# ywq/psnerf

Measured on AMD Instinct MI355X. Metric: ray-samples/sec (train step) on BEAR stage2, higher is better.
Workload: dtype f32

## Files before the change

include/psnerf_hip.h:

```cpp
#ifndef PSNERF_HIP_H
#define PSNERF_HIP_H

#include <stdint.h>

#ifdef __cplusplus
extern "C" {
#endif

#define PSN_OK 0
#define PSN_E_ARG (-1)
#define PSN_E_LAUNCH (-2)
#define PSN_E_UNSUPPORTED (-3)

const char* psn_last_error(void);
int psn_version(void);

int psn_composite_fwd(const float* alpha, const float* rgb, int64_t n_rays, int n_samples, int white_bg,
                      float* weights, float* rgb_out, float* acc_out, void* stream);
int psn_composite_bwd(const float* alpha, const float* rgb, const float* d_rgb_out, const float* d_acc_out,
                      int64_t n_rays, int n_samples, int white_bg, float* d_alpha, float* d_rgb, void* stream);

int psn_pe_encode(const float* x, int64_t n, int n_freqs, float scale, float* out, int out_stride, void* stream);
int psn_app_input(const float* p, const float* v, const float* normal, int64_t n, int n_freqs, float* out, void* stream);

// ... 161 lines not shown
    const float* const* mask_ptrs; const float* const* aux2_ptrs; float* const* save2_ptrs;
    const float* act_init; int64_t act_init_rows; const float* rk_coef; const float* rk_basis; int rk_k; const uint32_t* dump_tiles;
    int64_t n_rows; float* out; const float* live_count; int64_t live_period;
} PsnMlpLaunch;
typedef struct { int chain, width16, src, trim, from_a, x3, tb_lds, pm_groups; int64_t blocks, pm_period; } PsnMlpPath;
int psn_mlp_launch(const PsnMlpDesc* desc, const float* packed_w, const float* packed_b, const PsnMlpLaunch* launch, PsnMlpPath* path,
                   void* stream);
int psn_mlp_last_path(PsnMlpPath* path);
int psn_mlp_block_order(int point_major);

#define PSN_SCATTER_MAX_ITEMS 16
typedef struct {
    const float* rows;
    float* dense;
    int64_t row_stride, col_stride;
    int B, C;
    float fill;
} PsnScatterItem;
int psn_scatter_rows(int n_items, const PsnScatterItem* items, const int* inv, int64_t N, int64_t Ns, void* stream);
int psn_gather_rows(int n_items, const PsnScatterItem* items, const int64_t* idx, int64_t N, int64_t Ns, void* stream);
int psn_gather_rows_valid(int n_items, const PsnScatterItem* items, const int64_t* idx, const int* inv, int64_t N, int64_t Ns, void* stream);

int psn_secant_step(const float* occ, float tau, float* d_pred, float* d_low, float* d_high, float* f_low, float* f_high,
                    const float* origin, const float* dir, float* p_mid, int64_t n, void* stream);

int psn_first_crossing(const float* occ, const float* far, const float* u, const float* omu, float near, float tau,
                       int64_t n_rays, int n_steps, float* bracket, int* flags, void* stream);

int psn_shadow_points(const float* surf, const float* ldir, int64_t n_surf, int n_lights, int n_steps, float lnear, float lfar,
                      const float* u, const float* omu, float box, float* pts, int64_t* rows, unsigned long long* counter,
                      void* stream);

int psn_mlp_infer_pe(const PsnMlpDesc* desc, const float* packed_w, const float* packed_b, const float* points, int64_t n_rows,
                     int pe_octaves, float pe_scale, float* out, void* stream);
int psn_mlp_infer_pe_indirect(const PsnMlpDesc* desc, const float* packed_w, const float* packed_b, const float* points,
                              int64_t capacity, const long long* n_rows_dev, const int64_t* out_rows, int pe_octaves,
                              float pe_scale, float* out, void* stream);

int psn_march_sweep(const PsnMlpDesc* desc, const float* packed_w, const float* packed_b, const float* origin, const float* dir,
                    const float* far, const float* u, const float* omu, float near, int64_t n_rays, int n_steps, float tau,
                    int pe_octaves, float pe_scale, int* skip, unsigned long long* n_blocks, float* occ, void* stream);

int psn_root_find(const PsnMlpDesc* desc, const float* packed_w, const float* packed_b, const float* origin, const float* dir,
                  const float* bracket, int64_t n_rays, float tau, int n_iter, int pe_octaves, float pe_scale, float* d_out,
                  void* stream);

int psn_stage2_loss_fwd(const float* rgb, const float* rgb_gt, int L, const float* alb, const float* alb_j, const float* wgt,
                        const float* wgt_j, int nb, const float* vis, const float* vis_gt, int V, const float* nrm,
                        const float* nrm_gt, const float* nrm_j, const unsigned char* mask_a, const unsigned char* mask_b,
                        int64_t N, int l2, const float* inv_denom, const float* weight, const float* count_dev, float* partial,
                        float* out, void* stream);
int psn_stage2_loss_bwd(const float* g_total, const float* rgb, const float* rgb_gt, int L, float k_rgb, float* d_rgb,
                        const float* alb, const float* alb_j, float k_alb, float* d_alb, float* d_alb_j, const float* wgt,
                        const float* wgt_j, int nb, float k_wgt, float* d_wgt, float* d_wgt_j, const float* vis, const float* vis_gt,
                        int V, float k_vis, float* d_vis, const float* nrm, const float* nrm_gt, const float* nrm_j, float k_nrm,
                        float k_nrmj, float* d_nrm, float* d_nrm_j, const unsigned char* mask_a, const unsigned char* mask_b,
                        int64_t N, int l2, const float* count_dev, void* stream);

int psn_stage1_loss_partial_floats(void);
int psn_stage1_loss_fwd(const float* rgb, const float* rgb_gt, const float* diff, const unsigned char* hit, const float* normal,
                        const float* normal_gt, const unsigned char* norm_mask, const float* acc, const float* mask_gt,
                        const unsigned char* mask_valid, int64_t N, int64_t n_rays, const float* weights, float* partial,
                        float* sums, float* terms, void* stream);
int psn_stage1_loss_terms(const float* sums, int64_t n_rays, const float* weights, int has_grad, int has_norm, int has_mask,
                          float* terms, void* stream);
int psn_stage1_loss_bwd(const float* g_loss, const float* sums, const float* rgb, const float* rgb_gt, const unsigned char* hit,
                        const float* normal, const float* normal_gt, const unsigned char* norm_mask, const float* acc,
                        const float* mask_gt, const unsigned char* mask_valid, int64_t N, int64_t n_rays, const float* weights,
                        float* d_rgb, float* d_diff, float* d_normal, float* d_acc, void* stream);
int psn_surface_normals_fwd(const float* g, const unsigned char* hit, int64_t N, float eps, float* norm_pred, float* diff,
                            void* stream);
int psn_surface_normals_bwd(const float* g, const unsigned char* hit, int64_t N, float eps, const float* d_norm_pred,
                            const float* d_diff, float* dg, void* stream);

#define PSN_PAIR_SUMS_MAX_V 16
#define PSN_PAIR_SUMS_MAX_CHUNKS 2048
int psn_pair_sums(const float* x, int V, int64_t Ns, int C, float* sx, float* sl_part, int* n_chunks, void* stream);
#define PSN_PAIR_GROUP_MAX 4
typedef struct { const float* x; float* sx; float* dWl; float* bias; } PsnPairSumsItem;
int64_t psn_pair_sums_group_workspace(int n_items, int V, int64_t Ns, int C);
int psn_pair_sums_group(int n_items, const PsnPairSumsItem* items, int V, int64_t Ns, int C, const float* pe_l, int64_t ld_pe, int n_pe,
                        int64_t ld_w, float* workspace, void* stream);

#define PSN_ROW_ADAM_MAX 4
typedef struct {
    float* param; const float* grad; float* exp_avg; float* exp_avg_sq;
    int64_t rows; int cols;
    float one_minus_beta1, one_minus_beta2, eps, step_size;
} PsnRowAdamItem;
int psn_row_adam(int n_items, const PsnRowAdamItem* items, const int64_t* idx, int n_idx, void* stream);
int psn_row_adam_dev(int n_items, const PsnRowAdamItem* items, const int64_t* idx, int n_idx, const float* step_sizes_dev, void* stream);

int psn_normalize_rows_fwd(const float* x, int64_t n, float eps, float* y, void* stream);
int psn_normalize_rows_bwd(const float* x, const float* g, int64_t n, float eps, float* dx, void* stream);
int psn_light_rows_fwd(const float* dir_table, const float* int_table, const int64_t* idx, int n_idx, float eps, float* dir_out,
                       float* int_out, void* stream);
int psn_light_rows_bwd(const float* dir_table, const int64_t* idx, int n_idx, int64_t n_rows, float eps, const float* g_dir,
                       const float* g_int, float* d_dir_table, float* d_int_table, void* stream);
int psn_camera_rays(const float* uv, const float* pose, const float* intrinsics, const int64_t* idx, int64_t n, float scale,
                    float* out, void* stream);
int psn_stage1_rays(const float* pix, const float* camera_mat, int k_ld, const float* world_mat, float radius2, int64_t n,
                    float* cam, float* rays, float* far, void* stream);
int psn_surface_points(const float* d_pred, const int* flags, const float* cam, const float* rays, int64_t n, float* d_i,
                       float* dists, unsigned char* obj_mask, float* points, void* stream);
int psn_stage1_targets(const float* pix, int64_t n, int h, int w, const float* img, const float* mask, const float* mask_valid,
                       const float* normal, const float* norm_mask, const float* world_mat, int use_angle, float cos_thresh,
                       float* rgb_gt, float* mask_gt, unsigned char* mask_valid_out, float* normal_gt,
                       unsigned char* norm_mask_out, void* stream);
#define PSN_COPY2D_MAX 24
typedef struct {
    const float* src; int64_t ld_src;
    float* dst; int64_t ld_dst;
    int rows, cols;
} PsnCopy2dItem;
int psn_copy2d_group(int n_items, const PsnCopy2dItem* items, void* stream);
#define PSN_COPY_BYTES_MAX 24
typedef struct { const void* src; void* dst; int64_t n_bytes; int aligned; } PsnCopyBytesItem;
int psn_copy_bytes_group(int n_items, const PsnCopyBytesItem* items, void* stream);
int psn_mask_count(const unsigned char* mask_a, const unsigned char* mask_b, int64_t n, float* out, void* stream);
int psn_surface_index(const unsigned char* mask, int64_t n, int64_t cap, int64_t* idx, float* count, void* stream);
int psn_inverse_index(const int64_t* idx, int64_t ns, int64_t n_pix, int* inv, const float* count, void* stream);
typedef struct {
    const void* images; int image_type; const float* lut;
    const unsigned char* object_mask; const unsigned char* surface_mask;
    const float* points; const float* normal; const float* visibility; const float* vis_plus; const float* light_direction;
    int64_t hw; int width;
    const int64_t* lidx; int n_lights;
    const int64_t* pix; int64_t pix0; int64_t n;
    const int64_t* vidx; int n_vis;
    float* rgb; unsigned char* object_mask_out; unsigned char* surface_mask_out; float* uv; float* points_out; float* normal_out;
    float* visibility_out; float* vis_train_gt; int64_t* sampling_idx_out; float* light_direction_out;
} PsnViewBatch;
int psn_view_batch(const PsnViewBatch* b, void* stream);
#define PSN_ADAM_MAX_SEGS 16
typedef struct {
    int64_t offset, grad_offset, n;
    float neg_step_size;
    float bias_correction2_sqrt;
} PsnAdamSeg;
int psn_adam_flat(float* param, const float* grad, float* exp_avg, float* exp_avg_sq, int n_segs, const PsnAdamSeg* segs,
                  float one_minus_beta1, float beta2, float one_minus_beta2, float eps, void* stream);
int psn_adam_flat_dev(float* param, const float* grad, float* exp_avg, float* exp_avg_sq, int n_segs, const PsnAdamSeg* segs,
                      float one_minus_beta1, float beta2, float one_minus_beta2, float eps, const float* seg_scalars_dev, void* stream);

#define PSN_WN_MAX_ITEMS 16
typedef struct {
    const float* v;
    const float* g;
    float* w;
    const float* dw;
    float* dv;
    float* dg;
    int rows, cols;
    float scale;
} PsnWnItem;
int psn_weight_norm_fwd(int n_items, const PsnWnItem* items, void* stream);
int psn_weight_norm_bwd(int n_items, const PsnWnItem* items, void* stream);

typedef struct {
    int32_t n_hidden;
    int32_t n_out;
    int32_t out_act;
    int32_t reserved;
    uint8_t has_in[PSN_MLP_MAX_LAYERS + 4];
} PsnBf16Desc;

// ... 132 lines not shown
```

psnerf_amd/csrc/gemm.hip:

```cpp
#include "common.h"

namespace psn {

constexpr int BM = 128, BK = 16, LDA = BM + 4, EPI_LD = 68;

struct GemmArgs {
    int64_t M;
    int N, K;
    const float* A;
    int64_t lda;
    const float* B;
    int64_t ldb;
    float* C;
    int64_t ldc;
    const float* bias;
    int epi;
    const float* aux_in;
    int64_t ld_aux_in;
    const float* aux_in2;
    int64_t ld_aux_in2;
    float* aux_out;
    int64_t ld_aux_out;
    int k_chunk;
    int tiles_n;
    int64_t n_tiles;
    int split_k;
    int a_vec, b_vec;
    int c_vec, auxin_vec, auxin2_vec, auxout_vec;
    int64_t split_stride;
    float* colsum;
    const float* A2;
    int64_t lda2;
    const float* B2;
    int64_t ldb2;
    int seg_splits;
    int b_div, b_mod;
    const float* Bt2;
    int64_t ldbt2;
    int b2_div, b2_mod, b_split;
};

__device__ __forceinline__ int fastdiv24(int k, int d) {
    int q = (int)((float)k * __builtin_amdgcn_rcpf((float)d));
    const int r = k - q * d;
    q += (r >= d ? 1 : 0) - (r < 0 ? 1 : 0);
    return q;
}

template <bool KCONTIG, int ROWS>
__device__ __forceinline__ void fetch_tile(const float* __restrict__ src, int64_t ld, int64_t row0, int64_t n_rows,
                                           int k0, int k_end, int vec_ok, int tid, float4 (&v)[ROWS / 64],
                                           int k_div = 0, int k_mod = 0, const float* __restrict__ src2 = nullptr,
                                           int64_t ld2 = 0, int k_div2 = 0, int k_mod2 = 0, int col_split = 0) {
#pragma unroll
    for (int u = 0; u < ROWS / 64; ++u) {
        int f = tid + 256 * u;
        float4 x = make_float4(0.f, 0.f, 0.f, 0.f);
        if (KCONTIG) {
            int r = f >> 2, kq = (f & 3) * 4;
            int64_t row = row0 + r;
            int k = k0 + kq;
            if (row < n_rows) {
                const float* p = src + row * ld + k;
                if (vec_ok && k + 3 < k_end) {
                    x = *reinterpret_cast<const float4*>(p);
                } else {
                    if (k + 0 < k_end) x.x = p[0];
                    if (k + 1 < k_end) x.y = p[1];
                    if (k + 2 < k_end) x.z = p[2];
                    if (k + 3 < k_end) x.w = p[3];
                }
            }
        } else {
            int kk = f / (ROWS / 4), rq = (f % (ROWS / 4)) * 4;
            int k = k0 + kk;
            int64_t row = row0 + rq;
            if (k < k_end) {
                const bool second = col_split > 0 && row >= col_split;
                const int kd = second ? k_div2 : k_div, km = second ? k_mod2 : k_mod;
                int ks = k;
                if (kd > 0) {
                    if (k_end <= (1 << 24)) {
                        if (kd > 1) ks = fastdiv24(k, kd);
// ... 201 lines not shown
#pragma unroll
            for (int e = 0; e < 4; ++e) {
                float x = vv[e];
                switch (epi) {
                    case PSN_EPI_NONE: break;
                    case PSN_EPI_BIAS: x = x + bb[e]; break;
                    case PSN_EPI_BIAS_RELU: x = fmaxf(x + bb[e], 0.0f); break;
                    case PSN_EPI_BIAS_SOFTPLUS: { float sp, sg; softplus100_sig(x + bb[e], sp, sg); x = sp; o2[e] = sg; break; }
                    case PSN_EPI_MUL_AUX: x = x * a1[e]; break;
                    case PSN_EPI_MUL_POS: x = a1[e] > 0.0f ? x : 0.0f; break;
                    case PSN_EPI_BIAS_SIGMOID: x = sigmoidf_(x + bb[e]); break;
                    case PSN_EPI_ACCUM: x = cin[e] + x; break;
                    case PSN_EPI_MUL2: o2[e] = x * a2[e]; x = x * a1[e]; break;
                    case PSN_EPI_SOFTPLUS_BWD: x = a1[e] * (x + 100.0f * a2[e] * (1.0f - a1[e])); break;
                    case PSN_EPI_MUL_AUX_RAW: o2[e] = x; x = x * a1[e]; break;
                    default: break;
                }
                vv[e] = x;
            }
            if (full4 && g.c_vec) *reinterpret_cast<float4*>(cp) = make_float4(vv[0], vv[1], vv[2], vv[3]);
            else { for (int e = 0; e < 4; ++e) if (nbase + e < g.N) cp[e] = vv[e]; }
            if (has_o2) {
                float* op = g.aux_out + m * g.ld_aux_out + nbase;
                if (full4 && g.auxout_vec) *reinterpret_cast<float4*>(op) = make_float4(o2[0], o2[1], o2[2], o2[3]);
                else { for (int e = 0; e < 4; ++e) if (nbase + e < g.N) op[e] = o2[e]; }
            }
        }
        __builtin_amdgcn_fence(__ATOMIC_ACQ_REL, "wavefront");
        __builtin_amdgcn_wave_barrier();
    }
    }
}

template <bool TA, bool TB, int NT>
__global__ __launch_bounds__(256) void gemm_kernel(GemmArgs g) {
    __shared__ __attribute__((aligned(16))) float lds_raw[GemmLds<NT>::FLOATS];
    gemm_tile<TA, TB, NT>(g, blockIdx.x, lds_raw);
}

constexpr int kMaxGroup = PSN_GEMM_TN_MAX_ITEMS;
struct GroupedArgs {
    int n;
    int64_t block_start[kMaxGroup + 1];
    GemmArgs g[kMaxGroup];
};
__global__ __launch_bounds__(256) void gemm_tn_grouped_kernel(GroupedArgs gg) {
    __shared__ __attribute__((aligned(16))) float lds_raw[GemmLds<2>::FLOATS];
    int i = 0;
    while (i + 1 < gg.n && (int64_t)blockIdx.x >= gg.block_start[i + 1]) ++i;
    const GemmArgs g = gg.g[i];
    const int64_t bid = (int64_t)blockIdx.x - gg.block_start[i];
    if (bid >= g.n_tiles * (int64_t)g.split_k) return;
    gemm_tile<true, false, 2>(g, bid, lds_raw);
}

template <int NU>
__device__ __forceinline__ void fetch_tile256(const float* __restrict__ src, int64_t ld, int n_rows, int k0, int k_end,
                                              int tid, float4 (&v)[NU]) {
    const int rqc = min((tid & 63) * 4, ((n_rows - 1) >> 2) << 2);
    const int wave = __builtin_amdgcn_readfirstlane(tid >> 6);
#pragma unroll
    for (int u = 0; u < NU; ++u) {
        const int kc = min(k0 + wave + 4 * u, k_end - 1);
        const float* row = src + (int64_t)kc * ld;
        v[u] = *reinterpret_cast<const float4*>(row + rqc);
    }
}
template <int NU>
__device__ __forceinline__ void mask_tile256(int n_rows, int k0, int k_end, int tid, float4 (&v)[NU]) {
    const int rq = (tid & 63) * 4;
    const int wave = __builtin_amdgcn_readfirstlane(tid >> 6);
    const bool c0 = rq + 0 < n_rows, c1 = rq + 1 < n_rows, c2 = rq + 2 < n_rows, c3 = rq + 3 < n_rows;
#pragma unroll
    for (int u = 0; u < NU; ++u) {
        const bool kin = k0 + wave + 4 * u < k_end;
        v[u].x = (kin && c0) ? v[u].x : 0.f;
        v[u].y = (kin && c1) ? v[u].y : 0.f;
        v[u].z = (kin && c2) ? v[u].z : 0.f;
        v[u].w = (kin && c3) ? v[u].w : 0.f;
    }
}

constexpr int T256 = 256, T256_LD = T256 + 4, TK = 32, T256_BUF = 2 * TK * T256_LD;
__global__ __launch_bounds__(256, 1) void gemm_tn256_grouped_kernel(GroupedArgs gg) {
    extern __shared__ __attribute__((aligned(16))) float lds256[];
    int gi = 0;
    while (gi + 1 < gg.n && (int64_t)blockIdx.x >= gg.block_start[gi + 1]) ++gi;
    const GemmArgs g = gg.g[gi];
    const int split = (int)((int64_t)blockIdx.x - gg.block_start[gi]);
    if (split >= g.split_k) return;
    const int tid = threadIdx.x;
    const int lane = tid & 63, wave = tid >> 6;
    const int wr = wave >> 1, wc = wave & 1;
    const int li = lane & 31, lh = lane >> 5;
    const bool seg2 = split >= g.seg_splits;
    const float* Ap = seg2 ? g.A2 : g.A;
    const float* Bp = seg2 ? g.B2 : g.B;
    const int64_t lda = seg2 ? g.lda2 : g.lda, ldb = seg2 ? g.ldb2 : g.ldb;
    const int k_begin = (seg2 ? split - g.seg_splits : split) * g.k_chunk;
    const int k_end = min(g.K, k_begin + g.k_chunk);
    const int nt = (k_end - k_begin + TK - 1) / TK;

    floatx16 acc[4][4];
#pragma unroll
    for (int i = 0; i < 4; ++i)
#pragma unroll
        for (int n = 0; n < 4; ++n)
#pragma unroll
            for (int r = 0; r < 16; ++r) acc[i][n][r] = 0.f;
    float4 ra[2][8], rb[2][8];
    const bool do_cs = g.colsum != nullptr && !seg2;
    float4 cs = make_float4(0.f, 0.f, 0.f, 0.f);
#define T_FETCH(T, S)                                                                            \
    fetch_tile256(Ap, lda, (int)g.M, k_begin + (T) * TK, k_end, tid, ra[S]);                     \
    fetch_tile256(Bp, ldb, g.N, k_begin + (T) * TK, k_end, tid, rb[S]);
#define T_STORE(BUF, S, T)                                                                       \
    mask_tile256((int)g.M, k_begin + (T) * TK, k_end, tid, ra[S]);                               \
    mask_tile256(g.N, k_begin + (T) * TK, k_end, tid, rb[S]);                                    \
    if (do_cs) {                                                                                 \
        _Pragma("unroll") for (int u2_ = 0; u2_ < 8; u2_ += 2) {                                 \
            cs.x += ra[S][u2_].x + ra[S][u2_ + 1].x; cs.y += ra[S][u2_].y + ra[S][u2_ + 1].y;    \
            cs.z += ra[S][u2_].z + ra[S][u2_ + 1].z; cs.w += ra[S][u2_].w + ra[S][u2_ + 1].w;    \
        }                                                                                        \
    }                                                                                            \
    _Pragma("unroll") for (int u_ = 0; u_ < 8; ++u_) {                                           \
        *reinterpret_cast<float4*>(lds256 + (BUF) * T256_BUF + ((tid >> 6) + 4 * u_) * T256_LD + (tid & 63) * 4) = ra[S][u_]; \
        *reinterpret_cast<float4*>(lds256 + (BUF) * T256_BUF + TK * T256_LD + ((tid >> 6) + 4 * u_) * T256_LD + (tid & 63) * 4) = rb[S][u_]; \
    }
    const int wave_u = __builtin_amdgcn_readfirstlane(tid >> 6);
    const int rq_ = (tid & 63) * 4;
    const bool am0 = rq_ + 0 < (int)g.M, am1 = rq_ + 1 < (int)g.M, am2 = rq_ + 2 < (int)g.M, am3 = rq_ + 3 < (int)g.M;
    const bool bm0 = rq_ + 0 < g.N, bm1 = rq_ + 1 < g.N, bm2 = rq_ + 2 < g.N, bm3 = rq_ + 3 < g.N;
    const int rqa = min(rq_, (((int)g.M - 1) >> 2) << 2), rqb = min(rq_, ((g.N - 1) >> 2) << 2);
    float4 cs01 = make_float4(0.f, 0.f, 0.f, 0.f);
#define T_ITEM(BUF, S, T, J, MASKED, BD)                                                         \
    if (!((BD) && (J) >= 8)) {                                                                   \
        constexpr int u_ = (J) & 7;                                                              \
        constexpr bool isb_ = (J) >= 8;                                                          \
        float4& x_ = isb_ ? rb[S][u_] : ra[S][u_];                                               \
        if (MASKED) {                                                                            \
            const bool kin_ = k_begin + ((T) + 1) * TK + wave_u + 4 * u_ < k_end;                \
            x_.x = (kin_ && (isb_ ? bm0 : am0)) ? x_.x : 0.f;                                    \
            x_.y = (kin_ && (isb_ ? bm1 : am1)) ? x_.y : 0.f;                                    \
            x_.z = (kin_ && (isb_ ? bm2 : am2)) ? x_.z : 0.f;                                    \
            x_.w = (kin_ && (isb_ ? bm3 : am3)) ? x_.w : 0.f;                                    \
        }                                                                                        \
        if (!isb_ && do_cs) {                                                                    \
            if ((u_ & 1) == 0) cs01 = x_;                                                        \
            else { cs.x += cs01.x + x_.x; cs.y += cs01.y + x_.y; cs.z += cs01.z + x_.z; cs.w += cs01.w + x_.w; } \
        }                                                                                        \
        *reinterpret_cast<float4*>(lds256 + (BUF) * T256_BUF + (isb_ ? TK * T256_LD : 0) + (wave_u + 4 * u_) * T256_LD + rq_) = x_; \
        const int kc_ = min(k_begin + ((T) + 3) * TK + wave_u + 4 * u_, k_end - 1);             \
        x_ = *reinterpret_cast<const float4*>((isb_ ? Bp + (int64_t)kc_ * ldb + rqb : Ap + (int64_t)kc_ * lda + rqa)); \
    }
#define T_STEP(T, S, MASKED, BD)                                                                 \
    {                                                                                            \
        __builtin_amdgcn_sched_barrier(0);                                                       \
        if (BD) { T_DMA_B(((T) + 1) & 1, (T) + 1) __builtin_amdgcn_sched_barrier(0); }           \
        const float* As = lds256 + ((T) & 1) * T256_BUF + wr * 128 + li;                         \
        const float* Bs = lds256 + ((T) & 1) * T256_BUF + TK * T256_LD + wc * 128 + li;          \
        float pa[2][4], pb[2][4];                                                                \
        _Pragma("unroll") for (int i = 0; i < 4; ++i) pa[0][i] = As[lh * T256_LD + i * 32];      \
        _Pragma("unroll") for (int n = 0; n < 4; ++n) pb[0][n] = Bs[lh * T256_LD + n * 32];      \
        __builtin_amdgcn_sched_barrier(0);                                                       \
        T_PAIR(T, S, 0, MASKED, BD) T_PAIR(T, S, 1, MASKED, BD) T_PAIR(T, S, 2, MASKED, BD) T_PAIR(T, S, 3, MASKED, BD)  \
        T_PAIR(T, S, 4, MASKED, BD) T_PAIR(T, S, 5, MASKED, BD) T_PAIR(T, S, 6, MASKED, BD) T_PAIR(T, S, 7, MASKED, BD)  \
        T_PAIR(T, S, 8, MASKED, BD) T_PAIR(T, S, 9, MASKED, BD) T_PAIR(T, S, 10, MASKED, BD) T_PAIR(T, S, 11, MASKED, BD)  \
        T_PAIR(T, S, 12, MASKED, BD) T_PAIR(T, S, 13, MASKED, BD) T_PAIR(T, S, 14, MASKED, BD) T_PAIR(T, S, 15, MASKED, BD)  \
                                                          \
        if (BD) asm volatile("s_waitcnt vmcnt(8)" ::: "memory");                                 \
        lds_barrier();  \
    }
#define T_PAIR(T, S, J, MASKED, BD)                                                              \
// ... 16 lines not shown
        __builtin_amdgcn_sched_barrier(0);                                                       \
    }
#define T_DMA_B(BUF, T)                                                                          \
    _Pragma("unroll") for (int u_ = 0; u_ < 8; ++u_) {                                           \
        const int kc_ = min(k_begin + (T) * TK + wave_u + 4 * u_, k_end - 1);                    \
        lds_dma_16<0>(Bp + (int64_t)kc_ * ldb, lds_addr(lds256 + (BUF) * T256_BUF + TK * T256_LD + (wave_u + 4 * u_) * T256_LD), \
                      (unsigned)(tid & 63) * 16u);                                               \
    }
    int t = 0;
    if (g.N == T256) {
        T_DMA_B(0, 0)
        fetch_tile256(Ap, lda, (int)g.M, k_begin, k_end, tid, ra[0]);
        mask_tile256((int)g.M, k_begin, k_end, tid, ra[0]);
        if (do_cs) {
#pragma unroll
            for (int u2_ = 0; u2_ < 8; u2_ += 2) {
                cs.x += ra[0][u2_].x + ra[0][u2_ + 1].x; cs.y += ra[0][u2_].y + ra[0][u2_ + 1].y;
                cs.z += ra[0][u2_].z + ra[0][u2_ + 1].z; cs.w += ra[0][u2_].w + ra[0][u2_ + 1].w;
            }
        }
#pragma unroll
        for (int u_ = 0; u_ < 8; ++u_)
            *reinterpret_cast<float4*>(lds256 + ((tid >> 6) + 4 * u_) * T256_LD + (tid & 63) * 4) = ra[0][u_];
        fetch_tile256(Ap, lda, (int)g.M, k_begin + TK, k_end, tid, ra[0]);
        fetch_tile256(Ap, lda, (int)g.M, k_begin + 2 * TK, k_end, tid, ra[1]);
        asm volatile("s_waitcnt vmcnt(16)" ::: "memory");
        __syncthreads();
        for (; t + 3 < nt; t += 2) {
            T_STEP(t, 0, false, true)
            T_STEP(t + 1, 1, false, true)
        }
        for (; t + 1 < nt; t += 2) {
            T_STEP(t, 0, true, true)
            T_STEP(t + 1, 1, true, true)
        }
        if (t < nt) T_STEP(t, 0, true, true)
    } else {
        T_FETCH(0, 0)
        T_STORE(0, 0, 0)
        T_FETCH(1, 0)
        T_FETCH(2, 1)
        __syncthreads();
        for (; t + 3 < nt; t += 2) {
            T_STEP(t, 0, false, false)
            T_STEP(t + 1, 1, false, false)
        }
        for (; t + 1 < nt; t += 2) {
            T_STEP(t, 0, true, false)
            T_STEP(t + 1, 1, true, false)
        }
        if (t < nt) T_STEP(t, 0, true, false)
    }
#undef T_DMA_B
#undef T_STEP
#undef T_PAIR
#undef T_ITEM
#undef T_FETCH
#undef T_STORE
    if (do_cs) {
        float4* red = reinterpret_cast<float4*>(lds256);
        red[wave * 64 + lane] = cs;
        __syncthreads();
        if (tid < 64) {
            const float4 a = red[tid], b = red[64 + tid], c = red[128 + tid], d = red[192 + tid];
            const float v[4] = {(a.x + b.x) + (c.x + d.x), (a.y + b.y) + (c.y + d.y), (a.z + b.z) + (c.z + d.z), (a.w + b.w) + (c.w + d.w)};
            float* dst = g.colsum + (int64_t)split * g.M + 4 * tid;
#pragma unroll
            for (int e = 0; e < 4; ++e)
                if (4 * tid + e < g.M) dst[e] = v[e];
        }
    }
    float* Cw = g.C + (int64_t)split * g.split_stride;
#pragma unroll
    for (int i = 0; i < 4; ++i)
#pragma unroll
        for (int n = 0; n < 4; ++n) {
            const int col = wc * 128 + n * 32 + li;
#pragma unroll
            for (int r = 0; r < 16; ++r) {
                const int row = wr * 128 + i * 32 + (r & 3) + 8 * (r >> 2) + 4 * lh;
                if (row < g.M && col < g.N) Cw[(int64_t)row * g.N + col] = acc[i][n][r];
            }
        }
}

typedef __bf16 gbf16x8 __attribute__((ext_vector_type(8)));
typedef __bf16 gbf16x2 __attribute__((ext_vector_type(2)));
typedef float gfloatx2 __attribute__((ext_vector_type(2)));
constexpr int XK = 16, X_ROW = 48, X_PLANE = T256 * X_ROW, X_OPND = 3 * X_PLANE, X_BUF = 2 * X_OPND;
__device__ __forceinline__ int x3g_cvt2(float a, float b) {
    gfloatx2 f;
    f[0] = a; f[1] = b;
    return __builtin_bit_cast(int, __builtin_convertvector(f, gbf16x2));
}
__device__ __forceinline__ void x3g_split2(float a, float b, int& hi, int& mid, int& lo) {
    hi = x3g_cvt2(a, b);
    const float ra = a - __builtin_bit_cast(float, hi << 16), rb = b - __builtin_bit_cast(float, hi & (int)0xFFFF0000);
    mid = x3g_cvt2(ra, rb);
    lo = x3g_cvt2(ra - __builtin_bit_cast(float, mid << 16), rb - __builtin_bit_cast(float, mid & (int)0xFFFF0000));
}
template <int NP>
__global__ __launch_bounds__(512, 1) void gemm_tn256_x3_grouped_kernel(GroupedArgs gg) {
    constexpr int NPL = NP == 6 ? 3 : NP == 3 ? 2 : 1;
    extern __shared__ __attribute__((aligned(16))) unsigned char ldsx[];
    int gi = 0;
    while (gi + 1 < gg.n && (int64_t)blockIdx.x >= gg.block_start[gi + 1]) ++gi;
    const GemmArgs g = gg.g[gi];
    const int split = (int)((int64_t)blockIdx.x - gg.block_start[gi]);
    if (split >= g.split_k) return;
    const int tid = threadIdx.x;
    const int lane = tid & 63, wave = __builtin_amdgcn_readfirstlane(tid >> 6);
    const int wr = wave >> 2, wc = wave & 3;
    const int kb = wave & 3, half = wave >> 2;
    const int li = lane & 31, lh = lane >> 5;
    const bool seg2 = split >= g.seg_splits;
    const float* Ap = seg2 ? g.A2 : g.A;
    const float* Bp = seg2 ? g.B2 : g.B;
    const int64_t lda = seg2 ? g.lda2 : g.lda, ldb = seg2 ? g.ldb2 : g.ldb;
    const int k_begin = (seg2 ? split - g.seg_splits : split) * g.k_chunk;
    const int k_end = min(g.K, k_begin + g.k_chunk);
    const int nt = (k_end - k_begin + XK - 1) / XK;

    floatx16 acc[4][2];
#pragma unroll
    for (int i = 0; i < 4; ++i)
#pragma unroll
        for (int n = 0; n < 2; ++n)
#pragma unroll
            for (int r = 0; r < 16; ++r) acc[i][n][r] = 0.f;
    float ra[2][2][4], rb[2][2][4];
    int ca[2], cb[2];
#pragma unroll
    for (int e = 0; e < 2; ++e) {
        ca[e] = min(lane + 64 * (2 * half + e), (int)g.M - 1);
        cb[e] = min(lane + 64 * (2 * half + e), g.N - 1);
    }
    const bool do_cs = g.colsum != nullptr && !seg2;
    float cs[2] = {0.f, 0.f};
    auto fetch = [&](int t, float (&va)[2][4], float (&vb)[2][4]) __attribute__((always_inline)) {
#pragma unroll
        for (int j = 0; j < 4; ++j) {
            const int kc = min(k_begin + t * XK + 4 * kb + j, k_end - 1);
            const float* arow = Ap + (int64_t)kc * lda;
            const float* brow = Bp + (int64_t)kc * ldb;
#pragma unroll
            for (int e = 0; e < 2; ++e) { va[e][j] = arow[ca[e]]; vb[e][j] = brow[cb[e]]; }
        }
    };
    auto stage = [&](int t, int buf, float (&va)[2][4], float (&vb)[2][4]) __attribute__((always_inline)) {
#pragma unroll
        for (int j = 0; j < 4; ++j) {
            const bool kin = k_begin + t * XK + 4 * kb + j < k_end;
#pragma unroll
            for (int e = 0; e < 2; ++e) { va[e][j] = kin ? va[e][j] : 0.f; vb[e][j] = kin ? vb[e][j] : 0.f; }
        }
#pragma unroll
        for (int e = 0; e < 2; ++e) cs[e] += (va[e][0] + va[e][1]) + (va[e][2] + va[e][3]);
        unsigned char* base = ldsx + buf * X_BUF;
#pragma unroll
        for (int e = 0; e < 2; ++e) {
            int h0, m0, l0, h1, m1, l1;
            x3g_split2(va[e][0], va[e][1], h0, m0, l0);
            x3g_split2(va[e][2], va[e][3], h1, m1, l1);
            unsigned char* d = base + (lane + 64 * (2 * half + e)) * X_ROW + kb * 8;
            *reinterpret_cast<int2*>(d) = make_int2(h0, h1);
            if constexpr (NPL >= 2) *reinterpret_cast<int2*>(d + X_PLANE) = make_int2(m0, m1);
// ... 131 lines not shown
    mask_tile64(g.N, k_begin + (T) * BK, k_end, tid, rb[S]);                                    \
    if (do_cs) {                                                                                \
        cs.x += (ra[S][0].x + ra[S][1].x) + (ra[S][2].x + ra[S][3].x); cs.y += (ra[S][0].y + ra[S][1].y) + (ra[S][2].y + ra[S][3].y); \
        cs.z += (ra[S][0].z + ra[S][1].z) + (ra[S][2].z + ra[S][3].z); cs.w += (ra[S][0].w + ra[S][1].w) + (ra[S][2].w + ra[S][3].w); \
    }                                                                                           \
    store_tile<false, T256>(lds + (BUF) * TALL_BUF, tid, ra[S]);                                \
    *reinterpret_cast<float4*>(lds + (BUF) * TALL_BUF + BK * T256_LD + (tid >> 4) * T64_LD + (tid & 15) * 4) = rb[S];
#define TL_STEP(T, S)                                                                           \
    {                                                                                           \
        __builtin_amdgcn_sched_barrier(0);                                                      \
        const float* As = lds + ((T) & 1) * TALL_BUF + wave * 64 + li;                          \
        const float* Bs = lds + ((T) & 1) * TALL_BUF + BK * T256_LD + li;                       \
        float pa[2][2], pb[2][2];                                                               \
        _Pragma("unroll") for (int i = 0; i < 2; ++i) pa[0][i] = As[lh * T256_LD + i * 32];     \
        _Pragma("unroll") for (int n = 0; n < 2; ++n) pb[0][n] = Bs[lh * T64_LD + n * 32];      \
        __builtin_amdgcn_sched_barrier(0);                                                      \
        _Pragma("unroll") for (int j = 0; j < 8; ++j) {                                         \
            if (j < 7) {                                                                        \
                _Pragma("unroll") for (int i = 0; i < 2; ++i) pa[(j + 1) & 1][i] = As[(2 * j + 2 + lh) * T256_LD + i * 32]; \
                _Pragma("unroll") for (int n = 0; n < 2; ++n) pb[(j + 1) & 1][n] = Bs[(2 * j + 2 + lh) * T64_LD + n * 32];  \
            }                                                                                   \
            _Pragma("unroll") for (int i = 0; i < 2; ++i)                                       \
                _Pragma("unroll") for (int n = 0; n < 2; ++n)                                   \
                    acc[i][n] = __builtin_amdgcn_mfma_f32_32x32x2f32(pa[j & 1][i], pb[j & 1][n], acc[i][n], 0, 0, 0); \
            __builtin_amdgcn_sched_barrier(0);                                                  \
        }                                                                                       \
        TL_STORE(((T) + 1) & 1, S, (T) + 1)                                                     \
        TL_FETCH((T) + 3, S)                                                                    \
        lds_barrier();      \
    }
    TL_FETCH(0, 0)
    TL_STORE(0, 0, 0)
    TL_FETCH(1, 0)
    TL_FETCH(2, 1)
    __syncthreads();
    int t = 0;
    for (; t + 1 < nt; t += 2) {
        TL_STEP(t, 0)
        TL_STEP(t + 1, 1)
    }
    if (t < nt) TL_STEP(t, 0)
#undef TL_STEP
#undef TL_STORE
#undef TL_FETCH
    if (do_cs) {
        float4* red = reinterpret_cast<float4*>(lds);
        red[wave * 64 + lane] = cs;
        __syncthreads();
        if (tid < 64) {
            const float4 a = red[tid], b = red[64 + tid], c = red[128 + tid], d = red[192 + tid];
            const float v[4] = {(a.x + b.x) + (c.x + d.x), (a.y + b.y) + (c.y + d.y), (a.z + b.z) + (c.z + d.z), (a.w + b.w) + (c.w + d.w)};
            float* dst = g.colsum + (int64_t)split * g.M + 4 * tid;
#pragma unroll
            for (int e = 0; e < 4; ++e)
                if (4 * tid + e < g.M) dst[e] = v[e];
        }
    }
    float* Cw = g.C + (int64_t)split * g.split_stride;
#pragma unroll
    for (int i = 0; i < 2; ++i)
#pragma unroll
        for (int n = 0; n < 2; ++n) {
            const int col = n * 32 + li;
#pragma unroll
            for (int r = 0; r < 16; ++r) {
                const int row = wave * 64 + i * 32 + (r & 3) + 8 * (r >> 2) + 4 * lh;
                if (row < g.M && col < g.N) Cw[(int64_t)row * g.N + col] = acc[i][n][r];
            }
        }
}

struct ReduceItem {
    const float* ws;
    const float* cs_ws;
    float* C;
    float* colsum;
    int64_t MN, ldc;
    int N, M, splits, cs_splits, accumulate, vec;
    int blocks;
};
struct GroupedReduceArgs {
    ReduceItem it[kMaxGroup];
};
__global__ __launch_bounds__(256) void grouped_reduce_kernel(GroupedReduceArgs ra) {
    const ReduceItem r = ra.it[blockIdx.y];
    __shared__ float4 red[8][32];
    const int b = blockIdx.x;
    if (b < r.blocks) {
        if (r.vec) {
            const int tx = threadIdx.x & 31, tz = threadIdx.x >> 5;
            const int64_t i = ((int64_t)b * 32 + tx) * 4;
            float4 s = make_float4(0.f, 0.f, 0.f, 0.f);
            if (i < r.MN) {
                const int per = (r.splits + 7) / 8;
                const int z0 = tz * per, z1 = min(r.splits, z0 + per);
#pragma unroll 8
                for (int z = z0; z < z1; ++z) {
                    const float4 v = *reinterpret_cast<const float4*>(r.ws + (int64_t)z * r.MN + i);
                    s.x += v.x; s.y += v.y; s.z += v.z; s.w += v.w;
                }
            }
            red[tz][tx] = s;
            __syncthreads();
            if (tz == 0 && i < r.MN) {
#pragma unroll
                for (int k = 1; k < 8; ++k) {
                    const float4 v = red[k][tx];
                    s.x += v.x; s.y += v.y; s.z += v.z; s.w += v.w;
                }
                const int64_t m = i / r.N, n = i % r.N;
                float4* cp = reinterpret_cast<float4*>(r.C + m * r.ldc + n);
                if (r.accumulate) {
                    const float4 c = *cp;
                    s.x += c.x; s.y += c.y; s.z += c.z; s.w += c.w;
                }
                *cp = s;
            }
        } else {
            const int64_t i = (int64_t)b * 256 + threadIdx.x;
            if (i < r.MN) {
                float s = 0.0f;
                for (int z = 0; z < r.splits; ++z) s += r.ws[(int64_t)z * r.MN + i];
                const int64_t m = i / r.N, n = i % r.N;
                float* cp = r.C + m * r.ldc + n;
                *cp = r.accumulate ? (*cp + s) : s;
            }
        }
    } else if (r.colsum != nullptr) {
        const int64_t m = (int64_t)(b - r.blocks) * 256 + threadIdx.x;
        if (m < r.M) {
            float s = 0.0f;
            for (int z = 0; z < r.cs_splits; ++z) s += r.cs_ws[(int64_t)z * r.M + m];
            r.colsum[m] = s;
        }
    }
}

__global__ __launch_bounds__(256) void splitk_reduce_kernel(const float* __restrict__ ws, int64_t MN, int N,
                                                            int64_t ldc, int splits, int accumulate,
                                                            float* __restrict__ C) {
    for (int64_t i = (int64_t)blockIdx.x * 256 + threadIdx.x; i < MN; i += (int64_t)gridDim.x * 256) {
        float s = 0.0f;
        for (int z = 0; z < splits; ++z) s += ws[(int64_t)z * MN + i];
        int64_t m = i / N, n = i % N;
        float* cp = C + m * ldc + n;
        *cp = accumulate ? (*cp + s) : s;
    }
}

__global__ __launch_bounds__(256) void splitk_reduce_vec_kernel(const float* __restrict__ ws, int64_t MN, int N,
                                                                int64_t ldc, int splits, int accumulate,
                                                                float* __restrict__ C) {
    __shared__ float4 red[8][32];
    const int tx = threadIdx.x & 31, tz = threadIdx.x >> 5;
    const int64_t i = ((int64_t)blockIdx.x * 32 + tx) * 4;
    float4 s = make_float4(0.f, 0.f, 0.f, 0.f);
    if (i < MN) {
        const int per = (splits + 7) / 8;
        const int z0 = tz * per, z1 = min(splits, z0 + per);
#pragma unroll 8
        for (int z = z0; z < z1; ++z) {
            const float4 v = *reinterpret_cast<const float4*>(ws + (int64_t)z * MN + i);
            s.x += v.x; s.y += v.y; s.z += v.z; s.w += v.w;
        }
    }
    red[tz][tx] = s;
    __syncthreads();
    if (tz == 0 && i < MN) {
#pragma unroll
        for (int k = 1; k < 8; ++k) {
            const float4 v = red[k][tx];
            s.x += v.x; s.y += v.y; s.z += v.z; s.w += v.w;
        }
        const int64_t m = i / N, n = i % N;
        float4* cp = reinterpret_cast<float4*>(C + m * ldc + n);
        if (accumulate) {
            const float4 c = *cp;
            s.x += c.x; s.y += c.y; s.z += c.z; s.w += c.w;
        }
        *cp = s;
    }
}

template <int NW>
__global__ __launch_bounds__(256) void colsum_partial_kernel(const float* __restrict__ X, const float* __restrict__ w,
                                                             int64_t ldw, int64_t M, int N, int64_t ldx,
                                                             int64_t rows_per_block, float* __restrict__ partial) {
    const int64_t r0 = (int64_t)blockIdx.x * rows_per_block;
    const int64_t r1 = min(M, r0 + rows_per_block);
    for (int n = threadIdx.x; n < N; n += 256) {
        if (NW == 0) {
            float s = 0.0f;
            for (int64_t m = r0; m < r1; ++m) s += X[m * ldx + n];
            partial[(int64_t)blockIdx.x * N + n] = s;
        } else {
            float s[NW > 0 ? NW : 1];
#pragma unroll
            for (int j = 0; j < NW; ++j) s[j] = 0.0f;
            for (int64_t m = r0; m < r1; ++m) {
                const float x = X[m * ldx + n];
#pragma unroll
                for (int j = 0; j < NW; ++j) s[j] += w[m * ldw + j] * x;
            }
#pragma unroll
            for (int j = 0; j < NW; ++j) partial[((int64_t)blockIdx.x * NW + j) * N + n] = s[j];
        }
    }
}
template <int NW>
__global__ __launch_bounds__(256) void colsum_partial_vec_kernel(const float* __restrict__ X, const float* __restrict__ w,
                                                                 int64_t ldw, int64_t M, int N, int64_t ldx,
                                                                 int64_t rows_per_block, float* __restrict__ partial) {
    constexpr int NW1 = NW > 0 ? NW : 1;
    __shared__ float4 red[3][NW1][64];
    const int c4 = (threadIdx.x & 63) * 4, rsub = threadIdx.x >> 6;
    const int64_t r0 = (int64_t)blockIdx.x * rows_per_block;
    const int64_t r1 = min(M, r0 + rows_per_block);
    float4 s[NW1];
#pragma unroll
    for (int j = 0; j < NW1; ++j) s[j] = make_float4(0.f, 0.f, 0.f, 0.f);
    if (c4 < N) {
#pragma unroll 4
        for (int64_t m = r0 + rsub; m < r1; m += 4) {
            const float4 x = *reinterpret_cast<const float4*>(X + m * ldx + c4);
#pragma unroll
            for (int j = 0; j < NW1; ++j) {
                const float wj = NW > 0 ? w[m * ldw + j] : 1.0f;
                if (NW > 0) { s[j].x += wj * x.x; s[j].y += wj * x.y; s[j].z += wj * x.z; s[j].w += wj * x.w; }
                else { s[j].x += x.x; s[j].y += x.y; s[j].z += x.z; s[j].w += x.w; }
            }
        }
    }
    if (rsub > 0) {
#pragma unroll
        for (int j = 0; j < NW1; ++j) red[rsub - 1][j][threadIdx.x & 63] = s[j];
    }
    __syncthreads();
    if (rsub == 0 && c4 < N) {
#pragma unroll
        for (int j = 0; j < NW1; ++j) {
            const float4 a = red[0][j][threadIdx.x], b = red[1][j][threadIdx.x], c = red[2][j][threadIdx.x];
            float4 t;
            t.x = (s[j].x + a.x) + (b.x + c.x); t.y = (s[j].y + a.y) + (b.y + c.y);
            t.z = (s[j].z + a.z) + (b.z + c.z); t.w = (s[j].w + a.w) + (b.w + c.w);
            *reinterpret_cast<float4*>(partial + ((int64_t)blockIdx.x * NW1 + j) * N + c4) = t;
        }
    }
}
__global__ __launch_bounds__(256) void colsum_final_kernel(const float* __restrict__ partial, int nblocks, int N, int NW,
                                                           int accumulate, float* __restrict__ out) {
    __shared__ float red[4];
    const int j = blockIdx.x / N, n = blockIdx.x % N;
    float s = 0.0f;
    for (int b = threadIdx.x; b < nblocks; b += 256) s += partial[((int64_t)b * NW + j) * N + n];
#pragma unroll
    for (int d = 32; d >= 1; d >>= 1) s += __shfl_xor(s, d, 64);
    if ((threadIdx.x & 63) == 0) red[threadIdx.x >> 6] = s;
    __syncthreads();
    if (threadIdx.x == 0) {
        float tot = (red[0] + red[1]) + (red[2] + red[3]);
        out[blockIdx.x] = accumulate ? out[blockIdx.x] + tot : tot;
    }
}

}

static void gemm_plan(int64_t M, int N, int K, uintptr_t A, int64_t lda, uintptr_t B, int64_t ldb, uintptr_t C, int64_t ldc,
                      uintptr_t aux_in, int64_t ld_aux_in, uintptr_t aux_in2, int64_t ld_aux_in2, uintptr_t aux_out,
                      int64_t ld_aux_out, int split_k, uintptr_t workspace, PsnGemmPlan* p) {
    using namespace psn;
    if (split_k < 1) split_k = 1;
    p->tiles_m = (M + BM - 1) / BM;
    int bn = N > 128 ? 256 : 128;
    if (bn == 256 && p->tiles_m * ((N + 255) / 256) * split_k < 2048) bn = 128;
    p->bn = bn;
    p->tiles_n = (N + bn - 1) / bn;
    p->a_vec = ((A & 15) == 0) && (lda % 4 == 0);
    p->b_vec = ((B & 15) == 0) && (ldb % 4 == 0);
    p->auxin_vec = aux_in && ((aux_in & 15) == 0) && (ld_aux_in % 4 == 0);
    p->auxin2_vec = aux_in2 && ((aux_in2 & 15) == 0) && (ld_aux_in2 % 4 == 0);
    p->auxout_vec = aux_out && ((aux_out & 15) == 0) && (ld_aux_out % 4 == 0);
    int kc = (K + split_k - 1) / split_k;
    kc = ((kc + BK - 1) / BK) * BK;
    split_k = (K + kc - 1) / kc;
    p->k_chunk = kc;
    p->split_k = split_k;
    const int64_t MN = M * (int64_t)N;
    p->c_vec = split_k > 1 ? ((workspace & 15) == 0) && (N % 4 == 0) && (MN % 4 == 0) : ((C & 15) == 0) && (ldc % 4 == 0);
    p->reduce = split_k == 1 ? 0 : (N % 4 == 0 && ldc % 4 == 0 && ((C | workspace) & 15) == 0 && MN / 128 < (1ll << 31)) ? 2 : 1;
    p->blocks = p->tiles_m * p->tiles_n * split_k;
    p->nt = (kc < K ? kc : K) / BK + ((kc < K ? kc : K) % BK ? 1 : 0);
    const int last = K - (split_k - 1) * kc;
    p->nt_last = (last + BK - 1) / BK;
    p->last_tile_rows = last - (p->nt_last - 1) * BK;
}

extern "C" int psn_gemm_plan(int64_t M, int N, int K, int64_t a_addr, int64_t lda, int64_t b_addr, int64_t ldb, int64_t c_addr,
                             int64_t ldc, int64_t aux_in_addr, int64_t ld_aux_in, int64_t aux_in2_addr, int64_t ld_aux_in2,
                             int64_t aux_out_addr, int64_t ld_aux_out, int split_k, int64_t workspace_addr, PsnGemmPlan* plan) {
    PSN_CHECK_ARG(plan, "gemm_plan: null plan");
    PSN_CHECK_ARG(M > 0 && N > 0 && K > 0, "gemm_plan: bad shape M=%lld N=%d K=%d", (long long)M, N, K);
    gemm_plan(M, N, K, (uintptr_t)a_addr, lda, (uintptr_t)b_addr, ldb, (uintptr_t)c_addr, ldc, (uintptr_t)aux_in_addr, ld_aux_in,
              (uintptr_t)aux_in2_addr, ld_aux_in2, (uintptr_t)aux_out_addr, ld_aux_out, split_k, (uintptr_t)workspace_addr, plan);
    return PSN_OK;
}

extern "C" int psn_gemm(int trans_a, int trans_b, int64_t M, int N, int K, const float* A, int64_t lda,
                        const float* B, int64_t ldb, float* C, int64_t ldc, const float* bias, int epilogue,
                        const float* aux_in, int64_t ld_aux_in, const float* aux_in2, int64_t ld_aux_in2,
                        float* aux_out, int64_t ld_aux_out, int split_k, float* workspace, float* colsum_a, void* stream) {
    using namespace psn;
    PSN_CHECK_ARG(A && B && C, "gemm: null operand");
    PSN_CHECK_ARG(colsum_a == nullptr || trans_a, "gemm: colsum_a needs trans_a (A stored [K][M])");
    PSN_CHECK_ARG(M >= 0 && N > 0 && K > 0, "gemm: bad shape M=%lld N=%d K=%d", (long long)M, N, K);
    PSN_CHECK_ARG(epilogue >= 0 && epilogue <= PSN_EPI_MUL_AUX_RAW, "gemm: unknown epilogue %d", epilogue);
    if (epilogue == PSN_EPI_MUL_AUX || epilogue == PSN_EPI_MUL_POS || epilogue >= PSN_EPI_MUL2) PSN_CHECK_ARG(aux_in, "gemm: epilogue needs aux_in");
    if (epilogue == PSN_EPI_MUL2 || epilogue == PSN_EPI_SOFTPLUS_BWD) PSN_CHECK_ARG(aux_in2, "gemm: epilogue needs aux_in2");
    if (epilogue == PSN_EPI_MUL2 || epilogue == PSN_EPI_MUL_AUX_RAW) PSN_CHECK_ARG(aux_out, "gemm: epilogue needs aux_out");
    if (epilogue >= PSN_EPI_BIAS && epilogue <= PSN_EPI_BIAS_SOFTPLUS) PSN_CHECK_ARG(bias, "gemm: epilogue needs bias");
    if (epilogue == PSN_EPI_BIAS_SIGMOID) PSN_CHECK_ARG(bias, "gemm: epilogue needs bias");
    if (split_k < 1) split_k = 1;
    if (split_k > 1) {
        PSN_CHECK_ARG(epilogue == PSN_EPI_NONE || epilogue == PSN_EPI_ACCUM, "gemm: split_k only with NONE/ACCUM epilogue");
        PSN_CHECK_ARG(workspace, "gemm: split_k needs workspace");
    }
    if (M == 0) return PSN_OK;
    hipStream_t st = (hipStream_t)stream;
    GemmArgs g;
    g.M = M; g.N = N; g.K = K; g.A = A; g.lda = lda; g.B = B; g.ldb = ldb; g.C = C; g.ldc = ldc;
    g.bias = bias; g.epi = epilogue; g.aux_in = aux_in; g.ld_aux_in = ld_aux_in; g.aux_out = aux_out;
    g.aux_in2 = aux_in2; g.ld_aux_in2 = ld_aux_in2;
    g.ld_aux_out = ld_aux_out;
    PsnGemmPlan pl;
    gemm_plan(M, N, K, (uintptr_t)A, lda, (uintptr_t)B, ldb, (uintptr_t)C, ldc, (uintptr_t)aux_in, ld_aux_in, (uintptr_t)aux_in2,
              ld_aux_in2, (uintptr_t)aux_out, ld_aux_out, split_k, (uintptr_t)workspace, &pl);
    PSN_CHECK_ARG(pl.tiles_m * pl.tiles_n < (1ll << 31), "gemm: too many tiles");
    const int bn = pl.bn;
    g.tiles_n = pl.tiles_n;
    g.n_tiles = pl.tiles_m * pl.tiles_n;
    g.a_vec = pl.a_vec; g.b_vec = pl.b_vec;
    g.auxin_vec = pl.auxin_vec; g.auxin2_vec = pl.auxin2_vec; g.auxout_vec = pl.auxout_vec;
    split_k = pl.split_k;
    g.k_chunk = pl.k_chunk;
    g.split_stride = 0;
// ... 202 lines not shown
            gg.block_start[gg.n++] = blocks;
            blocks += (g.n_tiles * g.split_k + 7) / 8 * 8;
        }
    }
    gg.block_start[gg.n] = blocks;
    gb.block_start[gb.n] = blocks_big;
    gt.block_start[gt.n] = blocks_tall;
    PSN_CHECK_ARG(ws_off <= workspace_floats, "gemm_tn_grouped: workspace too small (%lld floats needed)", (long long)ws_off);
    PSN_CHECK_ARG(blocks < (1ll << 31) && blocks_big < (1ll << 31) && blocks_tall < (1ll << 31), "gemm_tn_grouped: too many blocks");
    hipStream_t st = (hipStream_t)stream;
    if (gb.n > 0) {
        if (x3 && g_x3_products == 6) hipLaunchKernelGGL(gemm_tn256_x3_grouped_kernel<6>, dim3((unsigned)blocks_big), dim3(512), 2 * X_BUF, st, gb);
        else if (x3 && g_x3_products == 3) hipLaunchKernelGGL(gemm_tn256_x3_grouped_kernel<3>, dim3((unsigned)blocks_big), dim3(512), 2 * X_BUF, st, gb);
        else if (x3) hipLaunchKernelGGL(gemm_tn256_x3_grouped_kernel<1>, dim3((unsigned)blocks_big), dim3(512), 2 * X_BUF, st, gb);
        else hipLaunchKernelGGL(gemm_tn256_grouped_kernel, dim3((unsigned)blocks_big), dim3(256), T256_BUF * 2 * sizeof(float), st, gb);
        PSN_CHECK_LAUNCH("gemm_tn_grouped (256 x 256 tiles)");
    }
    if (gt.n > 0) {
        hipLaunchKernelGGL(gemm_tn_tall_grouped_kernel, dim3((unsigned)blocks_tall), dim3(256), 0, st, gt);
        PSN_CHECK_LAUNCH("gemm_tn_grouped (256 x 64 tiles)");
    }
    if (gg.n > 0) {
        hipLaunchKernelGGL(gemm_tn_grouped_kernel, dim3((unsigned)blocks), dim3(256), 0, st, gg);
        PSN_CHECK_LAUNCH("gemm_tn_grouped");
    }
    hipLaunchKernelGGL(grouped_reduce_kernel, dim3((unsigned)max_rblocks, (unsigned)n_items), dim3(256), 0, st, ra);
    PSN_CHECK_LAUNCH("gemm_tn_grouped reduce");
    return PSN_OK;
}

static void colsum_plan(uintptr_t X, int n_w, int64_t M, int N, int64_t ldx, uintptr_t workspace, PsnColsumPlan* p) {
    const int nw1 = n_w > 0 ? n_w : 1;
    int nblocks = (int)((M + 127) / 128);
    if (nblocks > 2048 / nw1) nblocks = 2048 / nw1;
    if (nblocks < 1) nblocks = 1;
    int64_t rpb = (M + nblocks - 1) / nblocks;
    if (rpb < 1) rpb = 1;
    p->nblocks = nblocks;
    p->rows_per_block = rpb;
    p->vec = N <= 256 && N % 4 == 0 && ldx % 4 == 0 && ((X | workspace) & 15) == 0;
}

extern "C" int psn_colsum_plan(int64_t x_addr, int n_w, int64_t M, int N, int64_t ldx, int64_t workspace_addr, PsnColsumPlan* plan) {
    PSN_CHECK_ARG(plan, "colsum_plan: null plan");
    PSN_CHECK_ARG(N > 0 && M >= 0 && n_w >= 0 && n_w <= 4, "colsum_plan: bad shape");
    colsum_plan((uintptr_t)x_addr, n_w, M, N, ldx, (uintptr_t)workspace_addr, plan);
    return PSN_OK;
}

extern "C" int psn_colsum(const float* X, const float* row_weight, int n_w, int64_t ldw, int64_t M, int N, int64_t ldx,
                          float* out, int accumulate, float* workspace, void* stream) {
    using namespace psn;
    PSN_CHECK_ARG(X && out && workspace, "colsum: null pointer");
    PSN_CHECK_ARG(N > 0 && M >= 0, "colsum: bad shape");
    PSN_CHECK_ARG(row_weight == nullptr ? n_w == 0 : (n_w >= 1 && n_w <= 4 && ldw >= n_w), "colsum: n_w=%d (1..4 with weights, 0 without)", n_w);
    hipStream_t st = (hipStream_t)stream;
    const int nw1 = n_w > 0 ? n_w : 1;
    PsnColsumPlan pl;
    colsum_plan((uintptr_t)X, n_w, M, N, ldx, (uintptr_t)workspace, &pl);
    const int nblocks = pl.nblocks;
    const int64_t rpb = pl.rows_per_block;
    const bool vec = pl.vec != 0;
    if (vec) {
        switch (n_w) {
            case 0: hipLaunchKernelGGL(colsum_partial_vec_kernel<0>, dim3(nblocks), dim3(256), 0, st, X, row_weight, ldw, M, N, ldx, rpb, workspace); break;
            case 1: hipLaunchKernelGGL(colsum_partial_vec_kernel<1>, dim3(nblocks), dim3(256), 0, st, X, row_weight, ldw, M, N, ldx, rpb, workspace); break;
            case 2: hipLaunchKernelGGL(colsum_partial_vec_kernel<2>, dim3(nblocks), dim3(256), 0, st, X, row_weight, ldw, M, N, ldx, rpb, workspace); break;
            case 3: hipLaunchKernelGGL(colsum_partial_vec_kernel<3>, dim3(nblocks), dim3(256), 0, st, X, row_weight, ldw, M, N, ldx, rpb, workspace); break;
            default: hipLaunchKernelGGL(colsum_partial_vec_kernel<4>, dim3(nblocks), dim3(256), 0, st, X, row_weight, ldw, M, N, ldx, rpb, workspace); break;
        }
    } else
    switch (n_w) {
        case 0: hipLaunchKernelGGL(colsum_partial_kernel<0>, dim3(nblocks), dim3(256), 0, st, X, row_weight, ldw, M, N, ldx, rpb, workspace); break;
        case 1: hipLaunchKernelGGL(colsum_partial_kernel<1>, dim3(nblocks), dim3(256), 0, st, X, row_weight, ldw, M, N, ldx, rpb, workspace); break;
        case 2: hipLaunchKernelGGL(colsum_partial_kernel<2>, dim3(nblocks), dim3(256), 0, st, X, row_weight, ldw, M, N, ldx, rpb, workspace); break;
        case 3: hipLaunchKernelGGL(colsum_partial_kernel<3>, dim3(nblocks), dim3(256), 0, st, X, row_weight, ldw, M, N, ldx, rpb, workspace); break;
        default: hipLaunchKernelGGL(colsum_partial_kernel<4>, dim3(nblocks), dim3(256), 0, st, X, row_weight, ldw, M, N, ldx, rpb, workspace); break;
    }
    PSN_CHECK_LAUNCH("colsum partial");
    hipLaunchKernelGGL(colsum_final_kernel, dim3(N * nw1), dim3(256), 0, st, workspace, nblocks, N, nw1, accumulate, out);
    PSN_CHECK_LAUNCH("colsum final");
    return PSN_OK;
}
```

psnerf_amd/csrc/loss.hip:

```cpp
#include "common.h"

namespace psn {

struct LossArgs {
    const float* rgb; const float* rgb_gt; int L;
    const float* alb; const float* alb_j;
    const float* wgt; const float* wgt_j; int nb;
    const float* vis; const float* vis_gt; int V;
    const float* nrm; const float* nrm_gt; const float* nrm_j;
    const unsigned char* mask_a; const unsigned char* mask_b;
    int64_t N;
    int l2;
    float* partial;
    const float* g_total;
    const float* count_dev;
    float k_rgb, k_alb, k_wgt, k_vis, k_nrm, k_nrmj;
    float* d_rgb; float* d_alb; float* d_alb_j; float* d_wgt; float* d_wgt_j; float* d_vis; float* d_nrm; float* d_nrm_j;
};

__device__ __forceinline__ float img_term(float a, float b, int l2) { const float d = a - b; return l2 ? d * d : fabsf(d); }
__device__ __forceinline__ float img_grad(float a, float b, int l2) {
    const float d = a - b;
    return l2 ? 2.0f * d : (d > 0.0f ? 1.0f : (d < 0.0f ? -1.0f : 0.0f));
}

__global__ __launch_bounds__(256) void stage2_loss_fwd_kernel(LossArgs a) {
    float s[6] = {0.f, 0.f, 0.f, 0.f, 0.f, 0.f};
    const int lc = (a.L + gridDim.y - 1) / gridDim.y;
    const int l0 = blockIdx.y * lc, l1 = min(a.L, l0 + lc);
    for (int64_t n = (int64_t)blockIdx.x * 256 + threadIdx.x; n < a.N; n += (int64_t)gridDim.x * 256) {
        if (!(a.mask_a[n] && a.mask_b[n])) continue;
        if (a.rgb != nullptr) {
#pragma unroll 4
            for (int l = l0; l < l1; ++l) {
                const float* p = a.rgb + ((int64_t)l * a.N + n) * 3;
                const float* q = a.rgb_gt + ((int64_t)l * a.N + n) * 3;
                s[0] += img_term(p[0], q[0], a.l2) + img_term(p[1], q[1], a.l2) + img_term(p[2], q[2], a.l2);
            }
        }
        if (blockIdx.y != 0) continue;
        if (a.alb != nullptr) {
#pragma unroll
            for (int c = 0; c < 3; ++c) s[1] += fabsf(a.alb[n * 3 + c] - a.alb_j[n * 3 + c]);
        }
        if (a.wgt != nullptr) {
            for (int k = 0; k < a.nb; ++k) s[2] += fabsf(a.wgt[n * a.nb + k] - a.wgt_j[n * a.nb + k]);
        }
        if (a.vis != nullptr) {
            for (int v = 0; v < a.V; ++v) s[3] += img_term(a.vis[((int64_t)v * a.N + n) * 3], a.vis_gt[(int64_t)v * a.N + n], a.l2);
        }
        if (a.nrm != nullptr) {
            const float gx = a.nrm_gt[n * 3], gy = a.nrm_gt[n * 3 + 1], gz = a.nrm_gt[n * 3 + 2];
            const float inv = 1.0f / fmaxf(sqrtf(gx * gx + gy * gy + gz * gz), 1e-12f);
            const float dx = a.nrm[n * 3] - gx * inv, dy = a.nrm[n * 3 + 1] - gy * inv, dz = a.nrm[n * 3 + 2] - gz * inv;
            s[4] += dx * dx + dy * dy + dz * dz;
            if (a.nrm_j != nullptr) {
#pragma unroll
                for (int c = 0; c < 3; ++c) s[5] += fabsf(a.nrm[n * 3 + c] - a.nrm_j[n * 3 + c]);
            }
        }
    }
    __shared__ float red[4][6];
#pragma unroll
    for (int i = 0; i < 6; ++i) {
        float v = s[i];
#pragma unroll
        for (int o = 32; o > 0; o >>= 1) v += __shfl_xor(v, o, 64);
        if ((threadIdx.x & 63) == 0) red[threadIdx.x >> 6][i] = v;
    }
    __syncthreads();
    if (threadIdx.x < 6)
        a.partial[((int64_t)blockIdx.y * gridDim.x + blockIdx.x) * 6 + threadIdx.x] = (red[0][threadIdx.x] + red[1][threadIdx.x]) + (red[2][threadIdx.x] + red[3][threadIdx.x]);
}

struct LossScale { float inv_denom[6]; float weight[6]; const float* count_dev; };
__global__ __launch_bounds__(256) void stage2_loss_final_kernel(const float* __restrict__ partial, int blocks, LossScale sc,
                                                               float* __restrict__ out) {
    __shared__ float red[32][8];
    const int i = threadIdx.x & 7, j = threadIdx.x >> 3;
    float s = 0.f;
    if (i < 6)
        for (int b = j; b < blocks; b += 32) s += partial[(int64_t)b * 6 + i];
    red[j][i] = s;
    __syncthreads();
    if (threadIdx.x < 8) {
        float tot = 0.f;
#pragma unroll
        for (int k = 0; k < 32; ++k) tot += red[k][threadIdx.x];
        const float cnt = sc.count_dev != nullptr ? sc.count_dev[0] : 1.0f;
        const float term = (threadIdx.x < 6 && cnt > 0.0f) ? tot * sc.inv_denom[threadIdx.x] / cnt : 0.f;
        if (threadIdx.x < 6) out[threadIdx.x] = term;
        float w = threadIdx.x < 6 ? sc.weight[threadIdx.x] * term : 0.f;
#pragma unroll
        for (int o = 4; o > 0; o >>= 1) w += __shfl_xor(w, o, 64);
        if (threadIdx.x == 0) out[6] = w;
    }
}

__global__ __launch_bounds__(256) void pair_sums_kernel(const float* __restrict__ x, int V, int64_t Ns, int C, int rows_per_block,
                                                        float* __restrict__ sx, float* __restrict__ sl_part) {
    const int cg = threadIdx.x & 63, rl = threadIdx.x >> 6;
    const int64_t n0 = (int64_t)blockIdx.x * rows_per_block, n1 = min(Ns, n0 + rows_per_block);
    const bool live = 4 * cg < C;
    float4 sl[PSN_PAIR_SUMS_MAX_V];
#pragma unroll
    for (int v = 0; v < PSN_PAIR_SUMS_MAX_V; ++v) sl[v] = make_float4(0.f, 0.f, 0.f, 0.f);
    if (live) {
        for (int64_t n = n0 + rl; n < n1; n += 4) {
            float4 acc = make_float4(0.f, 0.f, 0.f, 0.f);
#pragma unroll
            for (int v = 0; v < PSN_PAIR_SUMS_MAX_V; ++v) {
                if (v < V) {
                    const float4 t = *reinterpret_cast<const float4*>(x + ((int64_t)v * Ns + n) * C + 4 * cg);
                    acc.x += t.x; acc.y += t.y; acc.z += t.z; acc.w += t.w;
                    sl[v].x += t.x; sl[v].y += t.y; sl[v].z += t.z; sl[v].w += t.w;
                }
            }
            *reinterpret_cast<float4*>(sx + n * C + 4 * cg) = acc;
        }
#pragma unroll
        for (int v = 0; v < PSN_PAIR_SUMS_MAX_V; ++v)
            if (v < V) *reinterpret_cast<float4*>(sl_part + (((int64_t)blockIdx.x * 4 + rl) * V + v) * C + 4 * cg) = sl[v];
    }
}

struct PairGroupArgs { PsnPairSumsItem it[PSN_PAIR_GROUP_MAX]; int V; int64_t Ns; int C; int rows_per_block; int chunks; float* part;
                       const float* pe_l; int64_t ld_pe; int n_pe; int64_t ld_w;
                       int slices; float* part2; };
__global__ __launch_bounds__(256) void pair_group_sums_kernel(PairGroupArgs a) {
    const PsnPairSumsItem it = a.it[blockIdx.y];
    const int V = a.V, C = a.C;
    const int64_t Ns = a.Ns;
    const int cg = threadIdx.x & 63, rl = threadIdx.x >> 6;
    const int64_t n0 = (int64_t)blockIdx.x * a.rows_per_block, n1 = min(Ns, n0 + a.rows_per_block);
    const bool live = 4 * cg < C;
    float4 sl[PSN_PAIR_SUMS_MAX_V];
#pragma unroll
    for (int v = 0; v < PSN_PAIR_SUMS_MAX_V; ++v) sl[v] = make_float4(0.f, 0.f, 0.f, 0.f);
    if (live) {
        for (int64_t n = n0 + rl; n < n1; n += 4) {
            float4 acc = make_float4(0.f, 0.f, 0.f, 0.f);
#pragma unroll
            for (int v = 0; v < PSN_PAIR_SUMS_MAX_V; ++v) {
                if (v < V) {
                    const float4 t = *reinterpret_cast<const float4*>(it.x + ((int64_t)v * Ns + n) * C + 4 * cg);
                    acc.x += t.x; acc.y += t.y; acc.z += t.z; acc.w += t.w;
                    sl[v].x += t.x; sl[v].y += t.y; sl[v].z += t.z; sl[v].w += t.w;
                }
            }
            *reinterpret_cast<float4*>(it.sx + n * C + 4 * cg) = acc;
        }
    }
    __shared__ float4 red[3][64];
    float* dst = a.part + (((int64_t)blockIdx.y * a.chunks + blockIdx.x) * V) * C;
#pragma unroll
    for (int v = 0; v < PSN_PAIR_SUMS_MAX_V; ++v) {
        if (v < V) {
            __syncthreads();
            if (rl > 0) red[rl - 1][cg] = sl[v];
            __syncthreads();
            if (rl == 0 && live) {
                float4 t = sl[v];
#pragma unroll
                for (int q = 0; q < 3; ++q) { const float4 o = red[q][cg]; t.x += o.x; t.y += o.y; t.z += o.z; t.w += o.w; }
                *reinterpret_cast<float4*>(dst + (int64_t)v * C + 4 * cg) = t;
            }
        }
    }
}
__global__ __launch_bounds__(1024) void pair_group_final_kernel(PairGroupArgs a) {
    const PsnPairSumsItem it = a.it[blockIdx.y];
    const int V = a.V, C = a.C;
    const int c0 = blockIdx.x * 64;
    const int cl = threadIdx.x & 63, v = threadIdx.x >> 6;
    __shared__ float dzl[PSN_PAIR_SUMS_MAX_V][64];
    __shared__ float pel[PSN_PAIR_SUMS_MAX_V][64];
    int ch = 0, ch_end = a.chunks;
    if (a.slices > 1) {
        const int per = (a.chunks + a.slices - 1) / a.slices;
        ch = blockIdx.z * per;
        ch_end = min(a.chunks, ch + per);
    }
    float s = 0.0f;
    if (v < V && c0 + cl < C) {
        const float* p = a.part + ((int64_t)blockIdx.y * a.chunks * V + v) * C + c0 + cl;
        const int64_t step = (int64_t)V * C;
        for (; ch + 4 <= ch_end; ch += 4) {
            const float t0 = p[(int64_t)ch * step], t1 = p[(int64_t)(ch + 1) * step], t2 = p[(int64_t)(ch + 2) * step], t3 = p[(int64_t)(ch + 3) * step];
            s += t0; s += t1; s += t2; s += t3;
        }
        for (; ch < ch_end; ++ch) s += p[(int64_t)ch * step];
        if (a.slices > 1) a.part2[(((int64_t)blockIdx.y * a.slices + blockIdx.z) * V + v) * C + c0 + cl] = s;
    }
    if (a.slices > 1) return;
    dzl[v][cl] = s;
    pel[v][cl] = (v < V && cl < a.n_pe) ? a.pe_l[(int64_t)v * a.ld_pe + cl] : 0.0f;
    __syncthreads();
    for (int e = threadIdx.x; e < 64 * a.n_pe; e += 1024) {
        const int c = e / a.n_pe, k = e - c * a.n_pe;
        if (c0 + c < C) {
            float w = 0.0f;
            for (int u = 0; u < V; ++u) w += dzl[u][c] * pel[u][k];
            it.dWl[(int64_t)(c0 + c) * a.ld_w + k] = w;
        }
    }
    if (it.bias != nullptr && threadIdx.x < 64 && c0 + (int)threadIdx.x < C) {
        float b = 0.0f;
        for (int u = 0; u < V; ++u) b += dzl[u][threadIdx.x];
        it.bias[c0 + threadIdx.x] = b;
    }
}

__global__ __launch_bounds__(256) void stage2_loss_bwd_kernel(LossArgs a) {
    float g = a.g_total[0];
    if (a.count_dev != nullptr) {
        const float cnt = a.count_dev[0];
        g = cnt > 0.0f ? g / cnt : 0.0f;
    }
    const int lc = (a.L + gridDim.y - 1) / gridDim.y;
    const int l0 = blockIdx.y * lc, l1 = min(a.L, l0 + lc);
    for (int64_t n = (int64_t)blockIdx.x * 256 + threadIdx.x; n < a.N; n += (int64_t)gridDim.x * 256) {
        const bool m = a.mask_a[n] && a.mask_b[n];
        if (a.d_rgb != nullptr) {
            const float k = g * a.k_rgb;
#pragma unroll 4
            for (int l = l0; l < l1; ++l) {
                const int64_t o = ((int64_t)l * a.N + n) * 3;
#pragma unroll
                for (int c = 0; c < 3; ++c) a.d_rgb[o + c] = m ? k * img_grad(a.rgb[o + c], a.rgb_gt[o + c], a.l2) : 0.f;
            }
        }
        if (blockIdx.y != 0) continue;
        if (a.d_alb != nullptr) {
            const float k = g * a.k_alb;
#pragma unroll
            for (int c = 0; c < 3; ++c) {
                const float v = m ? k * img_grad(a.alb[n * 3 + c], a.alb_j[n * 3 + c], 0) : 0.f;
                a.d_alb[n * 3 + c] = v;
                a.d_alb_j[n * 3 + c] = -v;
            }
        }
        if (a.d_wgt != nullptr) {
            const float k = g * a.k_wgt;
            for (int q = 0; q < a.nb; ++q) {
                const float v = m ? k * img_grad(a.wgt[n * a.nb + q], a.wgt_j[n * a.nb + q], 0) : 0.f;
                a.d_wgt[n * a.nb + q] = v;
                a.d_wgt_j[n * a.nb + q] = -v;
            }
        }
        if (a.d_vis != nullptr) {
            const float k = g * a.k_vis;
// ... 210 lines not shown
```

psnerf_amd/hip.py:

```python
import ctypes
import os

import torch

from . import cabi

_HERE = os.path.dirname(os.path.abspath(__file__))
LIB_PATH = os.path.join(_HERE, 'libpsnerf_hip.so')

if not os.path.exists(LIB_PATH):
    raise ImportError(
        'psnerf_amd: %s is missing. Build it with `python -m psnerf_amd.build` (hipcc, gfx950). '
        'There is no fallback path.' % LIB_PATH)
_lib = ctypes.CDLL(LIB_PATH)

HEADER_PATH = os.path.join(_HERE, '..', 'include', 'psnerf_hip.h')
if not os.path.exists(HEADER_PATH):
    raise ImportError('psnerf_amd: %s is missing: the binding is derived from it. There is no fallback path.' % HEADER_PATH)

_constants, _structs, SIGNATURES = cabi.parse(HEADER_PATH)
globals().update({_k[len('PSN_'):]: _v for _k, _v in _constants.items()})
globals().update(_structs)
MAX_LAYERS = MLP_MAX_LAYERS
for _name, (_res, _args) in SIGNATURES.items():
# ... 858 lines not shown
def colsum_plan(X, n_w=0, workspace_addr=0):
    pl = PsnColsumPlan()
    _check(_lib.psn_colsum_plan(_addr(X), n_w, X.shape[0], X.shape[1], _ld(X), workspace_addr, ctypes.addressof(pl)), 'colsum_plan')
    return pl


def gemm_tn_grouped(items, split_k=None, x3=None):
    res = []
    K = items[0]['A'].shape[0]
    dev = items[0]['A'].device
    kinds = {id(it): ('big' if _tn_is_big(it) else ('tall' if _tn_is_tall(it) else 'tile')) for it in items}
    if split_k is None:
        work = 0
        for it in items:
            if kinds[id(it)] == 'tile':
                tiles = ((it['A'].shape[1] + 127) // 128) * ((it['B'].shape[1] + 127) // 128)
                work += tiles * (2 if it.get('A2') is not None else 1)
        want = max(1, (1024 + work - 1) // max(work, 1))
        min_rows = 512 if K >= 16384 else 128
        split_k = int(max(1, min(want, K // min_rows if K >= min_rows else 1, 256)))
    for c0 in range(0, len(items), GEMM_TN_MAX_ITEMS):
        chunk = items[c0:c0 + GEMM_TN_MAX_ITEMS]
        arr = (PsnGemmTnItem * len(chunk))()
        need = 0
        keep = []
        is_big = lambda it_: kinds[id(it_)] == 'big'
        n_big = sum((2 if it.get('A2') is not None else 1) for it in chunk if is_big(it))
        split_big = 1
        if n_big:
            want = max(1, min(256 // n_big, K // 256 if K >= 256 else 1))
            kc = -(-K // want)
            kc = (kc + 15) // 16 * 16
            split_big = -(-K // kc)
        n_tall = sum((2 if it.get('A2') is not None else 1) for it in chunk if kinds[id(it)] == 'tall')
        split_tall = 1
        if n_tall:
            want = max(1, min(256 // n_tall, K // 256 if K >= 256 else 1))
            kc = -(-K // want)
            kc = (kc + 15) // 16 * 16
            split_tall = -(-K // kc)
        for i, it in enumerate(chunk):
            M, N = _tn_shape(it, K)
            C = it.get('out')
            if C is None:
                C = torch.empty(M, N, device=dev, dtype=torch.float32)
            assert C.shape == (M, N)
            cs = torch.empty(M, device=dev, dtype=torch.float32) if it.get('colsum') else None
            A2 = it.get('A2')
            e = arr[i]
            _tn_fill(e, it, K, _mat_ptr)
            e.C, e.ldc = _mat_ptr(C, 'out'), _ld(C)
            e.colsum_a = None if cs is None else cs.data_ptr()
            sk = max(split_k, split_big) if is_big(it) else (max(split_k, split_tall) if kinds[id(it)] == 'tall' else split_k)
            need += (2 if A2 is not None else 1) * sk * M * N + sk * M + 16
            keep.append((C, cs))
        ws = workspace(need, dev)
        flops = sum(2.0 * (arr[i].k_rows or K) * arr[i].M * arr[i].N * (2 if chunk[i].get('A2') is not None else 1) for i in range(len(chunk)))
        use_x3 = WGRAD_X3 if x3 is None else bool(x3)
        with _Prof('gemm_tn_grouped', flops):
            _check((_lib.psn_gemm_tn_grouped_x3 if use_x3 else _lib.psn_gemm_tn_grouped)(
                len(chunk), ctypes.addressof(arr), K, split_k, ws.data_ptr(), ws.numel(), _stream()), 'gemm_tn_grouped')
        res += keep
    return res


def colsum(X, out=None, accumulate=False, row_weight=None):
    M, N = X.shape
    n_w, ldw, wp = 0, 0, None
    if row_weight is not None:
        w2 = row_weight if row_weight.dim() == 2 else row_weight.reshape(M, 1)
        assert w2.stride(1) == 1 and 1 <= w2.shape[1] <= 4
        n_w, ldw, wp = w2.shape[1], w2.stride(0), _mat_ptr(w2, 'row_weight')
    if out is None:
        out = torch.empty((n_w, N) if n_w else (N,), device=X.device, dtype=torch.float32)
    ws = workspace(2048 * N, X.device)
    xp = _mat_ptr(X, 'X')
    if M == 0:
        xp, wp = ws.data_ptr(), (ws.data_ptr() if n_w else None)
    _check(_lib.psn_colsum(xp, wp, n_w, ldw, M, N, _ld(X), out.data_ptr(), int(accumulate), ws.data_ptr(),
                           _stream()), 'colsum')
    return out


def mlp_pack_layer(W, n_mt, k_tiles, dst, transpose=False):
    assert W.dim() == 2 and W.stride(1) == 1 and W.is_cuda and W.dtype == torch.float32
    rows, cols = (W.shape[1], W.shape[0]) if transpose else (W.shape[0], W.shape[1])
    _check(_lib.psn_mlp_pack_layer(W.data_ptr(), W.stride(0), rows, cols, int(transpose), n_mt, k_tiles, dst.data_ptr(),
                                   _stream()), 'mlp_pack_layer')


def mlp_pack_layers(plan):
    for c0 in range(0, len(plan), PACK_MAX_ITEMS):
        chunk = plan[c0:c0 + PACK_MAX_ITEMS]
        arr = (PsnPackItem * len(chunk))()
        for e, item in zip(arr, chunk):
            W, transpose, n_mt, k_tiles, dst = item[:5]
            e.format = item[5] if len(item) > 5 else W_F32
            assert W.dim() == 2 and W.stride(1) == 1 and W.is_cuda and W.dtype == torch.float32
            assert dst.is_contiguous() and dst.numel() == n_mt * k_tiles * 1024
            rows, cols = (W.shape[1], W.shape[0]) if transpose else (W.shape[0], W.shape[1])
            e.W, e.dst, e.ldw = W.data_ptr(), dst.data_ptr(), W.stride(0)
            e.rows, e.cols, e.transpose, e.n_mt, e.k_tiles = rows, cols, int(transpose), n_mt, k_tiles
        _check(_lib.psn_mlp_pack_layers(len(chunk), ctypes.addressof(arr), _stream()), 'mlp_pack_layers')


class block_order(object):

    def __init__(self, order):
        assert order in ('point', 'row'), order
        self.order = order

    def __enter__(self):
        self.saved = _lib.psn_mlp_block_order(1 if self.order == 'point' else 0)
        return self

    def __exit__(self, *exc):
        _lib.psn_mlp_block_order(self.saved)
        return False


def mlp_infer(desc, packed_w, packed_b, tab_a, a_div, a_mod, tab_b, b_div, b_mod, n_rows, out=None, init_a=None,
              init_b=None, save=None, save_row0=0, mask=None, aux2=None, save2=None, act_init=None, macs_per_row=None,
              rank_init=None, save_tiles=None, save2_tiles=None, act_init_rows=None, live=None, save_bits=None, path=None):
    o, keep = PsnMlpLaunch(), []
    if save_tiles is not None or save2_tiles is not None:
        tiles_arr = (ctypes.c_uint32 * (2 * MAX_LAYERS))(*([0xFFFFFFFF] * (2 * MAX_LAYERS)))
        for base, lst in ((0, save_tiles), (MAX_LAYERS, save2_tiles)):
            for l, m in enumerate(lst or []):
                if m is not None:
                    tiles_arr[base + l] = int(m)
        keep.append(tiles_arr)
        o.dump_tiles = ctypes.addressof(tiles_arr)
    if rank_init is not None:
        rk_coef, rk_basis = rank_init
        o.rk_k = rk_k = rk_basis.shape[0]
        assert rk_coef.shape == (n_rows, rk_k) and rk_coef.is_contiguous() and rk_basis.is_contiguous() and 1 <= rk_k <= 4
        assert rk_basis.shape[1] == desc.init_stride, 'rank_init: the basis rows are init_stride floats'
        o.rk_coef, o.rk_basis = _tptr(rk_coef, 'rk_coef'), _tptr(rk_basis, 'rk_basis')
    if act_init is not None:
        o.act_init_rows = n_rows if act_init_rows is None else act_init_rows
        assert act_init.is_contiguous() and act_init.shape[0] >= o.act_init_rows, 'act_init: fewer rows than act_init_rows'
        o.act_init = _tptr(act_init, 'act_init')
    if out is None and desc.n_out > 0:
        out = torch.empty(n_rows, desc.n_out, device=packed_w.device, dtype=torch.float32)
    n_hidden = desc.n_layers - 1 if desc.n_out > 0 else desc.n_layers

    def ptr_array(lst, n, name, words=None):
        if lst is None:
            return None
        assert len(lst) == n, '%s: expected %d entries' % (name, n)
        is_words = lambda t: t.dtype == torch.int64 if words is None else words
        keep.append((ctypes.c_void_p * n)(*[None if t is None else (_bits_ptr(t, name) if is_words(t) else _tptr(t, name)) for t in lst]))
        return ctypes.addressof(keep[-1])

    o.mask_ptrs, o.aux2_ptrs, o.save2_ptrs = (ptr_array(lst, desc.n_layers, name) for lst, name in ((mask, 'mask'), (aux2, 'aux2'), (save2, 'save2')))
    o.save_ptrs, o.save_bits_ptrs = ptr_array(save, n_hidden, 'save', False), ptr_array(save_bits, n_hidden, 'save_bits', True)
    for t, b in zip(save or [], save_bits or []):
        assert b is None or (t is not None and b.shape == (t.shape[0], 4))
    if live is not None:
        cnt, period = live
        assert cnt.is_cuda and cnt.dtype == torch.float32 and cnt.numel() == 1 and int(period) >= 1
        o.live_count, o.live_period = cnt.data_ptr(), int(period)
    o.tab_a, o.a_div, o.a_mod = _tptr(tab_a, 'tab_a', allow_none=True), a_div, a_mod
    o.tab_b, o.b_div, o.b_mod = _tptr(tab_b, 'tab_b', allow_none=True), b_div, b_mod
    o.init_a, o.init_b = _tptr(init_a, 'init_a', allow_none=True), _tptr(init_b, 'init_b', allow_none=True)
    o.save_row0, o.n_rows, o.out = save_row0, n_rows, _tptr(out, 'out', allow_none=True)
# ... 612 lines not shown
```

psnerf_amd/ops.py:

```python
import collections

import torch

from . import fused, hip


HITS = collections.Counter()


def _hit(name):
    HITS[name] += 1


import os as _os0
STRICT = _os0.environ.get('PSN_STRICT', '0') == '1'
FALLBACKS = collections.Counter()


def fallback(name, tensor=None, why=''):
    if tensor is not None and not getattr(tensor, 'is_cuda', False):
        return
    FALLBACKS[name] += 1
    if STRICT:
        raise RuntimeError('psnerf_amd.ops.STRICT: %s left the fused engines on a device tensor%s' % (name, (' (' + why + ')') if why else ''))
# ... 445 lines not shown
            if need_w:
                dW[n - 1] = torch.zeros_like(Ws[n - 1])
                dW[n - 1][0] = hip.colsum(dR)

        g = d_out.contiguous()
        add_dW(n - 1, g, A[n - 1], with_bias=True)
        for l in range(n - 1, 0, -1):
            in_a = Ws[l].shape[1] - d_pe if l in skips else Ws[l].shape[1]
            g_prev = _buf(Q, in_a, dev)
            if sweep:
                hip.gemm(g, Ws[l][:, :in_a], epi=hip.EPI_SOFTPLUS_BWD, aux_in=S[l - 1], aux_in2=dS[l - 1], out=g_prev)
            else:
                hip.gemm(g, Ws[l][:, :in_a], epi=hip.EPI_MUL_AUX, aux_in=S[l - 1], out=g_prev)
            g = g_prev
            if need_p and (l - 1 == 0 or (l - 1) in skips):
                dz_pe[l - 1] = g
            add_dW(l - 1, g, A[l - 1], with_bias=True)
        if need_w:
            dW[0] = dW[0][:, :d_pe]
        d_p = None
        if need_p:
            sks = [l for l in sorted(dz_pe) if l > 0]
            first = sks[0] if sks else None
            d_p = hip.geo_point_grad(p, ctx.n_octaves, ctx.scale, dz_pe[0], W0p,
                                     dzs=None if first is None else dz_pe[first],
                                     ws=None if first is None else Ws[first][:, Ws[first].shape[1] - d_pe:],
                                     g_pe=sv[-1] if sweep else None, d_grad=d_grad.contiguous() if sweep else None)
            for l in sks[1:]:
                d_p = d_p + hip.geo_point_grad(p, ctx.n_octaves, ctx.scale, dz_pe[l], Ws[l][:, Ws[l].shape[1] - d_pe:])
        grads = []
        for l in range(n):
            grads += [dW[l], db[l]]
        return (d_p, None, None, None, None) + tuple(grads)


class MFShade(torch.autograd.Function):

    @staticmethod
    def forward(ctx, light_dir, view, normal, albedo, rough, light_int, vis, f0):
        _hit('MFShade')
        li_t, li_s = None, 0.0
        if torch.is_tensor(light_int):
            li_t = light_int.reshape(-1).expand(light_dir.shape[0]).contiguous() if light_int.numel() == 1 \
                else light_int.reshape(-1).contiguous()
        else:
            li_s = float(light_int)
        vis_f = None if vis is None else vis.reshape(-1).contiguous()
        args = (light_dir.contiguous(), view.contiguous(), normal.contiguous(), albedo.contiguous(),
                rough.reshape(-1).contiguous())
        rgb = hip.mf_shade_fwd(*args, li_t, li_s, f0, vis_f)
        ctx.save_for_backward(*args, *([li_t] if li_t is not None else []), *([vis_f] if vis_f is not None else []))
        ctx.has_li, ctx.has_vis, ctx.li_s, ctx.f0 = li_t is not None, vis_f is not None, li_s, f0
        ctx.li_shape = light_int.shape if torch.is_tensor(light_int) else None
        ctx.vis_shape = None if vis is None else vis.shape
        ctx.rough_shape = rough.shape
        return rgb

    @staticmethod
    def backward(ctx, g_rgb):
        sv = list(ctx.saved_tensors)
        light_dir, view, normal, albedo, rough = sv[:5]
        k = 5
        li_t = sv[k] if ctx.has_li else None
        k += 1 if ctx.has_li else 0
        vis_f = sv[k] if ctx.has_vis else None
        want_vis = ctx.has_vis and ctx.needs_input_grad[6]
        d_alb, d_r, d_n, d_vis, d_ld, d_li = hip.mf_shade_bwd(light_dir, view, normal, albedo, rough, li_t, ctx.li_s,
                                                              ctx.f0, vis_f, g_rgb.contiguous(), want_vis)
        if d_li is not None:
            n_li = 1
            for d in ctx.li_shape:
                n_li *= d
            d_li = d_li.sum().reshape(ctx.li_shape) if n_li == 1 else d_li.reshape(ctx.li_shape)
        if d_vis is not None:
            d_vis = d_vis.reshape(ctx.vis_shape)
        return d_ld, None, d_n, d_alb, d_r.reshape(ctx.rough_shape), d_li, d_vis, None


def mf_shade(light_dir, view, normal, albedo, rough, light_int, vis, f0):
    return MFShade.apply(light_dir, view, normal, albedo, rough, light_int, vis, f0)


RELU_SIGN_BITS = True


def _sign_bits(rows, n, device):
    return [torch.empty(rows, 4, device=device, dtype=torch.int64) for _ in range(n)]


class VisibilityPair(torch.autograd.Function):

    @staticmethod
    def launch(pe_x, pe_l, n_shade, in_cols, skip_at, params, need_grad, packed=None, live_count=None):
        Ws, bs = params[0::2], params[1::2]
        Ns, LV = pe_x.shape[0], pe_l.shape[0]
        V = LV - n_shade
        n = len(Ws)
        din_half = in_cols.numel() // 2
        with torch.no_grad():
            if packed is None:
                packed = fused.pack_relu_mlp(list(Ws), list(bs), din_half, din_half, skip_at)
            save = [torch.empty(V * Ns, 256, device=pe_x.device) for _ in range(n - 1)] if (need_grad and V > 0) else None
            bits = _sign_bits(V * Ns, n - 1, pe_x.device) if (save is not None and RELU_SIGN_BITS) else None
            out = packed(pe_x, LV * Ns, a_div=1, a_mod=Ns, tab_b=pe_l, b_div=Ns, b_mod=LV, save=save, save_row0=n_shade * Ns,
                         live=None if (live_count is None or Ns % 64 != 0) else (live_count, Ns),
                         save_bits=bits)
        return out, (save, bits) if save is not None else None

    @staticmethod
    def forward(ctx, pe_x, pe_l, n_shade, in_cols, skip_at, pre, *params):
        _hit('VisibilityPair')
        Ns, LV = pe_x.shape[0], pe_l.shape[0]
        V = LV - n_shade
        n = len(params) // 2
        need = any(ctx.needs_input_grad[6:])
        out, dumps = pre if pre is not None else VisibilityPair.launch(pe_x, pe_l, n_shade, in_cols, skip_at, params, need)
        save, bits = dumps if (need and dumps is not None) else (None, None)
        if save is not None:
            ctx.save_for_backward(pe_x, pe_l[n_shade:], in_cols, *save, *params)
        ctx.bits = bits
        ctx.n, ctx.skip_at, ctx.V, ctx.saved = n, skip_at, V, save is not None
        ctx.contiguous_cols = bool(getattr(in_cols, '_psn_contiguous_pair', False))
        vis, vis_t = out[:n_shade * Ns], out[n_shade * Ns:]
        ctx.mark_non_differentiable(vis)
        return vis, vis_t

    @staticmethod
    def backward(ctx, _g_vis, g):
        n, V = ctx.n, ctx.V
        if not ctx.saved or g is None:
            return (None,) * (6 + 2 * n)
        sv = ctx.saved_tensors
        pe_x, pe_lv, in_cols = sv[0], sv[1], sv[2]
        H = sv[3:3 + n - 1]
        Ws = sv[3 + n - 1::2]
        Ns = pe_x.shape[0]
        Q = V * Ns
        half = in_cols.numel() // 2
        cols_a, cols_b = in_cols[:half], in_cols[half:] - pe_x.shape[1]
        contiguous_cols = ctx.contiguous_cols
        grads = [None] * (2 * n)
        g = g.contiguous()

        bits = ctx.bits
        chain = fused.pack_relu_bwd(list(Ws), ctx.skip_at, bits=bits is not None, x3=CHAIN_X3)
        DZ = [torch.empty(Q, 256, device=g.device) for _ in range(n - 1)]
        chain(None, Q, a_div=1, a_mod=Q, rank_init=(g.reshape(Q, 1), Ws[n - 1].reshape(1, -1).contiguous()),
              mask=[(bits if bits is not None else H)[n - 2 - j] for j in range(n - 1)], save=DZ, save_row0=0)
        grads[2 * (n - 1)] = hip.colsum(H[n - 2], row_weight=g)
        grads[2 * (n - 1) + 1] = _rowsum_small(g)
        items = []
        where = []
        xl = {}
        for li in range(n - 2, -1, -1):
            dz = DZ[n - 2 - li]
            if li > 0:
                items.append(dict(A=dz, B=H[li - 1], colsum=True))
                where.append((li, 'w'))
            if li == 0 or li - 1 == ctx.skip_at:
                if V <= 16:
                    xl[li] = None
                else:
                    dz3 = dz.view(V, Ns, dz.shape[1])
                    dz_x, dz_l = dz3.sum(0), dz3.sum(1)
                    dWl = hip.gemm(dz_l, pe_lv.contiguous(), trans_a=True)
                    xl[li] = [dz_x, dWl, dz_l.sum(0) if li == 0 else None]
        grouped = [li for li in sorted(xl) if xl[li] is None]
        if grouped:
            pl = pe_lv.contiguous()
            for li, r in zip(grouped, hip.pair_sums_group([DZ[n - 2 - li] for li in grouped], V, Ns, pl, pl.shape[1],
                                                          [li == 0 for li in grouped])):
                xl[li] = list(r)
        lis = sorted(xl)
        for li, (C, _cs) in zip(lis, hip.gemm_tn_grouped([dict(A=xl[li][0], B=pe_x) for li in lis])):
            xl[li][0] = C
        parts = {}
        if items:
            for (li, kind), (C, cs) in zip(where, hip.gemm_tn_grouped(items)):
                parts[(li, kind)] = C
                if cs is not None:
                    grads[2 * li + 1] = cs
        for li in range(n - 1):
            blocks = [parts[(li, 'w')]] if (li, 'w') in parts else []
            if li in xl:
                dWx, dWl, cs0 = xl[li]
                blocks += [dWx[:, :half] if contiguous_cols else dWx[:, cols_a], dWl[:, :half] if contiguous_cols else dWl[:, cols_b]]
                if cs0 is not None:
                    grads[2 * li + 1] = cs0
            grads[2 * li] = blocks[0] if len(blocks) == 1 else torch.cat(blocks, dim=1)
        return (None, None, None, None, None, None) + tuple(grads)


CHAIN_X3 = False


class chain_precision(object):
    def __init__(self, mode):
        assert mode in ('fp32', 'bf16x3'), mode
        self.mode = mode

    def __enter__(self):
        global CHAIN_X3
        self.saved, CHAIN_X3 = CHAIN_X3, self.mode == 'bf16x3'
        return self

    def __exit__(self, *exc):
        global CHAIN_X3
        CHAIN_X3 = self.saved
        return False


class GeoFieldFused(torch.autograd.Function):

    @staticmethod
    def forward(ctx, p, n_octaves, scale, skips, with_grad, chains, feat_rows, *params):
        _hit('GeoFieldFused')
        Ws = [w for w in params[0::2]]
        n = len(Ws)
        p = p.contiguous()
        Q, dev = p.shape[0], p.device
        feat_rows = Q if feat_rows is None else int(feat_rows)
        assert 1 <= feat_rows <= Q
        d_pe = 3 + 6 * n_octaves
        d_a = chains['d_a']
        sk = skips[0]
        pe = hip.pe_encode(p, n_octaves, 64, scale)
        A = [torch.empty(Q, 256, device=dev) for _ in range(n - 1)]
        feat = torch.empty(Q, 256, device=dev)
        logit = chains['fwd'](pe, Q, save=A + [feat])
        A[sk - 1][:, d_a:] = pe[:, :d_pe]
        grad = None
        U = R = None
        if with_grad:
            U = [torch.empty(Q, 256, device=dev) for _ in range(n - 1)]
            r_sk = torch.empty(Q, 256, device=dev)
            w_row = Ws[n - 1][0:1, :].contiguous()
            t_sk = sum(1 << t for t in range(d_a // 16, (d_a + d_pe - 1) // 16 + 1))
            r0 = chains['sweep'](None, Q, a_div=1, a_mod=1, init_a_direct=w_row,
                                 mask=[A[n - 2 - j] for j in range(n - 1)] + [None],
                                 save=[U[n - 2 - j] for j in range(n - 1)],
                                 save2=[None] + [r_sk if n - 1 - j == sk else None for j in range(1, n - 1)] + [None],
                                 save2_tiles=[None] + [t_sk if n - 1 - j == sk else None for j in range(1, n - 1)] + [None])
            grad = hip.pe_encode_bwd(p, r0, n_octaves, scale, add=r_sk[:, d_a:d_a + d_pe])
        if any(ctx.needs_input_grad):
            ctx.meta = (n, sk, d_pe, d_a, n_octaves, scale, with_grad, chains, feat_rows)
            keep = [p, pe] + Ws + A
            if with_grad:
                keep += U
                if ctx.needs_input_grad[0]:
                    keep += [r0, r_sk]
            ctx.save_for_backward(*keep)
        if grad is None:
            grad = torch.zeros(Q, 3, device=dev)
            ctx.mark_non_differentiable(grad)
        return logit, (feat if feat_rows == Q else feat[:feat_rows]), grad

    @staticmethod
    def backward(ctx, d_logit, d_feat, d_grad):
        n, sk, d_pe, d_a, n_octaves, scale, with_grad, chains, feat_rows = ctx.meta
# ... 307 lines not shown
```

psnerf_amd/stage2/renderer.py:

```python
import contextlib
import os

import numpy as np
import torch
import torch.nn as nn
import torch.nn.functional as F

from .. import fused, hip, ops

PE_STRIDE = 64


def camera_rays(uv, pose, intrinsics):
    fx, fy = intrinsics[:, 0, 0], intrinsics[:, 1, 1]
    cx, cy = intrinsics[:, 0, 2], intrinsics[:, 1, 2]
    z = torch.ones_like(uv[:, :, 0])
    x = (uv[:, :, 0] - cx.unsqueeze(-1)) / fx.unsqueeze(-1) * z
    y = (uv[:, :, 1] - cy.unsqueeze(-1)) / fy.unsqueeze(-1) * z
    R = pose[:, :3, :3]
    d = x.unsqueeze(-1) * R[:, None, :, 0] + y.unsqueeze(-1) * R[:, None, :, 1] + z.unsqueeze(-1) * R[:, None, :, 2]
    return F.normalize(d, dim=2), pose[:, :3, 3]


class MLP(fused.PackCached, nn.Module):
# ... 170 lines not shown
        net = self.visibility_net
        if net.width != 256 or not net.linears[0].weight.is_cuda:
            return None
        return self._vis_pack('fp32', lambda prev, *net_args: fused.pack_relu_mlp(*net_args, reuse=prev))

    def _vis_pack(self, slot, build):
        net = self.visibility_net

        def make(prev):
            Ws, bs = net.weights()
            half = 3 + 6 * self.n_freqs
            return build(prev, list(Ws), list(bs), half, half, net._skip_index())
        return self.packs.get(slot, net.parameters(), make)

    def _vis_out_act(self):
        return hip.OUT_SIGMOID if self.visibility_net.final == 'sigmoid' else hip.OUT_NONE

    @torch.no_grad()
    def _visibility_rows_bf16(self, pe_x, pe_l):
        pack = self._vis_pack('bf16', lambda prev, *net_args: fused.pack_relu_mlp_bf16_grouped(*net_args, self._vis_out_act()))
        return pack(pe_x.to(torch.bfloat16), pe_l.contiguous())

    @torch.no_grad()
    def _visibility_rows_x3(self, pe_x, pe_l):
        pack = self._vis_pack('bf16x6', lambda prev, *net_args: fused.pack_relu_mlp_x3_grouped(*net_args, self._vis_out_act()))
        return pack(pe_x.contiguous(), pe_l.contiguous())

    @torch.no_grad()
    def _visibility_rows_b3(self, pe_x, pe_l):
        pack = self._vis_pack('bf16x3', lambda prev, *net_args: fused.pack_relu_mlp(
            *net_args, out_act=self._vis_out_act(), reuse=prev, x3=True))
        ns, nl = pe_x.shape[0], pe_l.shape[0]
        return pack(pe_x.contiguous(), nl * ns, a_div=1, a_mod=ns, tab_b=pe_l.contiguous(), b_div=ns, b_mod=nl)

    def _visibility_rows_lowp(self, mode, pe_x, pe_l):
        rows = {'bf16': self._visibility_rows_bf16, 'bf16x6': self._visibility_rows_x3, 'bf16x3': self._visibility_rows_b3}
        return rows[mode](pe_x, pe_l)

    def _memo(self, tag, input, fn):
        cache = self._eval_cache
        if cache is None or torch.is_grad_enabled():
            return fn()
        key = (tag,) + tuple((input[k].data_ptr(), input[k]._version) for k in ('points', 'surface_mask', 'uv')) \
            + self.packs.key(self.parameters())
        if key not in cache:
            cache[key] = fn()
        return cache[key]

    def _visibility_pair_launch(self, pe_x, light_dir, light_vis_train, live_count=None):
        a = self._visibility_pair_args(pe_x, light_dir, light_vis_train)
        need = any(p.requires_grad for p in a[5])
        return a, ops.VisibilityPair.launch(a[0], a[1], a[2], a[3], a[4], [p.detach() for p in a[5]], need,
                                            packed=self._visibility_prepack(), live_count=live_count)

    def _visibility_pair(self, pe_x, light_dir, light_vis_train, launched=None):
        if launched is not None:
            a, pre = launched
        else:
            a, pre = self._visibility_pair_args(pe_x, light_dir, light_vis_train), None
        return ops.VisibilityPair.apply(a[0], a[1], a[2], a[3], a[4], pre, *a[5])

    def forward(self, input, albedo_new=None, basis_new=None, noise=None):
        noise = noise or {}
        uv, pose, intr = input['uv'], input['pose'], input['intrinsics']
        object_mask = input['object_mask']
        device = uv.device
        surface_mask, points, normals = input['surface_mask'], input['points'], input['normal']
        idx = input.get('surface_idx')
        if idx is None:
            idx = surface_mask[0].nonzero(as_tuple=True)[0]
        ns = idx.shape[0]

        def gather(t):
            return t[0].index_select(0, idx)

        n_pix = points.shape[1]

        def scatter(dense, rows):
            return _Dense(dense.fill, dense.B, dense.C, rows)

        def ones3(b=1):
            return _Dense(1.0, b, 3)

        surf = gather(points).contiguous()
        out_n = {}
        normal_s = None
        pe_x = None
        vis_pair = None
        vis_bf16 = None
        side = None
        pair_ok = False
        if ns > 0 and self.visibility:
            lv0 = input.get('light_vis_train')
            ld0 = input['light_direction']
            pair_ok = (lv0 is not None and self.conf.get_bool('train.vis_rgb_detach', default=False)
                       and self.visibility_net.width == 256 and torch.is_grad_enabled()
                       and (self.light_vis_detach or not (ld0.requires_grad or lv0.requires_grad)))
            if pair_ok:
                pe_x = self._pe(surf, self.n_freqs)
                if self.overlap_small_nets and surf.is_cuda:
                    side = self._side.get(device)
                    if side is None:
                        side = self._side[device] = torch.cuda.Stream(device=device)
                    side.wait_stream(torch.cuda.current_stream(device))
                mode = 'bf16x3' if self.train_vis_bf16x3 else 'bf16x6' if self.train_vis_bf16x6 else 'bf16' if self.train_vis_bf16 else None
                if mode is not None:
                    pe_l0 = self._pe(ld0.detach(), self.n_freqs)
                    vis_bf16 = self._visibility_rows_lowp(mode, pe_x, pe_l0)
                    vis_pair = self._visibility_pair_launch(pe_x, ld0[:0], lv0)
                else:
                    vis_pair = self._visibility_pair_launch(pe_x, ld0, lv0, live_count=input.get('surface_count'))
        on_side = (lambda: torch.cuda.stream(side)) if side is not None else contextlib.nullcontext
        if self.normal_mlp:
            normal_pred = ones3()
            if ns > 0:
              with on_side():
                cols_n = self._cols(self.n_freqs_n, device)
                pe_n = (lambda: pe_x) if (pe_x is not None and self.n_freqs_n == self.n_freqs) else (lambda: self._pe(surf, self.n_freqs_n))
                if self.normal_jitter_std > 0 and torch.is_grad_enabled():
                    nz = noise.get('normal')
                    if nz is None:
                        nz = torch.empty_like(surf).normal_(0.0, self.normal_jitter_std)
                    pe_both_n = torch.cat([pe_n(), self._pe(surf + nz, self.n_freqs_n)], dim=0)
                    normal_s, nj = ops.SplitRows.apply(ops.normalize_rows(self.normal_net(pe_both_n, cols_n)), ns)
                    normal_pred = scatter(normal_pred, normal_s)
                    out_n['normal_jitter'] = scatter(ones3(), nj)
                else:
                    normal_s = self._memo('normal', input, lambda: ops.normalize_rows(self.normal_net(pe_n(), cols_n)))
                    normal_pred = scatter(normal_pred, normal_s)
                    if self.normal_jitter_std > 0:
                        nz = noise.get('normal')
                        if nz is None:
                            nz = torch.empty_like(surf).normal_(0.0, self.normal_jitter_std)
                        nj = self._memo('normal_jitter', input, lambda: ops.normalize_rows(
                            self.normal_net(self._pe(surf + nz, self.n_freqs_n), cols_n)))
                        out_n['normal_jitter'] = scatter(ones3(), nj)
            out_n['normal_pred'] = normal_pred

        sg = self.render_model == 'sgbasis'
        lnum = input['light_direction'].shape[0]
        rgb_values = ones3(lnum)
        albedo_values = ones3()
        rough_values = ones3(lnum) if sg else ones3()
        weight_values = _Dense(0.0, 1, self.nbasis) if sg else None
        vis_values = ones3(lnum)
        jitter = None
        vis_t_pre = None
        if ns > 0:
            normal = gather(normals) if not self.normal_mlp else normal_s
            with on_side():
                if (uv.is_cuda and uv.shape[0] == 1 and uv.dtype == torch.float32 and tuple(pose.shape[1:]) == (4, 4)
                        and tuple(intr.shape[1:]) == (4, 4)):
                    pts2c = hip.camera_rays(uv.contiguous(), pose.contiguous().float(), intr.contiguous().float(), idx, scale=-1.0)
                else:
                    ray_dirs, _ = camera_rays(uv, pose, intr)
                    pts2c = -gather(ray_dirs)
            light_dir = input['light_direction']
            cols = self._cols(self.n_freqs, device)
            if pe_x is None:
                pe_x = self._memo('pe_x', input, lambda: self._pe(surf, self.n_freqs))
            pe_j = None
            with on_side():
              if self.xyz_jitter_std > 0:
                nz = noise.get('xyz')
                if nz is None:
                    nz = torch.empty_like(surf).normal_(0.0, self.xyz_jitter_std)
# ... 24 lines not shown
                main.wait_stream(side)
                for t_ in (pts2c, normal_s, albedo_both if self.xyz_jitter_std > 0 else albedo, rough_both if self.xyz_jitter_std > 0 else rough,
                           weights if sg else None, out_n.get('normal_jitter').rows if 'normal_jitter' in out_n else None):
                    if torch.is_tensor(t_):
                        t_.record_stream(main)
            light_int = input.get('light_intensity', self.light_int)
            vis = None
            vis_for_rgb = None
            vis_t_pre = None
            if self.visibility:
                detach = self.conf.get_bool('train.vis_rgb_detach', default=False)
                if pair_ok:
                    if vis_bf16 is not None:
                        _none, vis_t_pre = self._visibility_pair(pe_x, light_dir[:0], lv0, launched=vis_pair)
                        vis = vis_bf16
                    else:
                        vis, vis_t_pre = self._visibility_pair(pe_x, light_dir, lv0, launched=vis_pair)
                else:
                    vis = self._visibility_rows(pe_x, light_dir, fused_ok=True)
                vis_for_rgb = vis.detach() if detach else vis
            if sg:
                rgb, spec = ops.sg_shade(light_dir, pts2c, normal, albedo, weights, self.sgbasis.lobe, light_int,
                                         vis_for_rgb, self.specular_rgb)
            else:
                rgb = ops.mf_shade(light_dir, pts2c, normal, albedo, rough, light_int, vis_for_rgb, self.f0)
            rgb_values = scatter(rgb_values, rgb)
            if vis is not None:
                vis_values = scatter(vis_values, vis.expand(rgb.shape))
            albedo_values = scatter(albedo_values, albedo)
            if sg:
                rough_values = scatter(rough_values, spec.expand(-1, 3))
            else:
                rough_values = scatter(rough_values, rough.expand(-1, 3))
            if self.xyz_jitter_std > 0:
                aj = scatter(ones3(), albedo_j)
                if sg:
                    rj = scatter(_Dense(1.0, 1, self.nbasis), rough_j)
                    r_ori = weight_values
                else:
                    rj = scatter(ones3(), rough_j.expand(-1, 3))
                    r_ori = rough_values
                jitter = {'albedo_values': albedo_values, 'albedo_jitter': aj,
                          'rough_values': r_ori, 'rough_jitter': rj}

        out = {
            'points': points, 'object_mask': object_mask, 'network_object_mask': surface_mask,
            'sg_rgb_values': rgb_values, 'normal_values': normals,
            'sg_diffuse_albedo_values': albedo_values, 'sg_specular_rgb_values': rough_values,
        }
        if jitter is not None:
            out.update(jitter)
        if self.normal_mlp:
            out.update(out_n)
        if self.visibility:
            out['visibility'] = vis_values
            if 'vis_train_gt' in input or 'light_vis_train' in input:
                lv = input['light_vis_train']
                vnum = lv.shape[0]
                vt = ones3(vnum)
                if ns > 0:
                    if vis_t_pre is not None:
                        vis_t = vis_t_pre
                    else:
                        train = torch.is_grad_enabled() and any(p.requires_grad for p in self.visibility_net.parameters())
                        vis_t = self._visibility_rows(pe_x, lv, fused_ok=not train)
                    vt = scatter(vt, vis_t.expand(-1, 3))
                out['vis_train'] = vt
        if sg:
            out['sg_weight'] = weight_values
        want = self._eval_outputs
        if want is not None:
            if 'sg_rgb_light_sum' in want:
                v = out['sg_rgb_values']
                rows_sum = v.rows.reshape(v.B, -1, v.C).sum(0) if v.rows is not None else None
                out['sg_rgb_light_sum'] = (rows_sum, idx if v.rows is not None else None, v.fill * v.B)
            out = {k: v for k, v in out.items() if k in want}
        lazy = {}
        for v in out.values():
            if isinstance(v, _Dense):
                lazy[id(v)] = v
        with_rows = [v for v in lazy.values() if v.rows is not None]
        done = {}
        if with_rows:
            if idx.is_cuda and idx.dtype == torch.int64:
                inv = hip.inverse_index(idx.contiguous(), n_pix, count=input.get('surface_count'))
            else:
                inv = torch.full((n_pix,), -1, dtype=torch.int32, device=device)
                inv[idx] = torch.arange(ns, dtype=torch.int32, device=device)
            specs = tuple((v.B, v.C, v.fill) for v in with_rows)
            dense = ops.ScatterRows.apply(idx, inv, specs, *[v.rows for v in with_rows])
            for v, d in zip(with_rows, dense):
                done[id(v)] = d
        for v in lazy.values():
            if v.rows is None:
                done[id(v)] = torch.full((v.B, n_pix, v.C), v.fill, device=device)
        for k in list(out.keys()):
            if isinstance(out[k], _Dense):
                out[k] = done[id(out[k])]
        return out
```

Before: 112.8 million.

## Co-schedule weight-grad GEMM tiles with column-sum and pair-sum side work in one launch

Adds a fused wgrad_sides kernel. It runs the big 256x256 split-K weight-gradient GEMM tiles alongside the column-sum and pair-sum reductions, with a fraction of the CUs set aside for the side work. A single finish kernel then does the split-K reduction and the side finalisation. This replaces several separate small launches that underuse the GPU with one partitioned launch plus one finish launch. The renderer also computes the inverse index earlier so it can be reused. The cost is more complex planning and a possible imbalance between the tile blocks and the side blocks.

New measurement: 113.4 million, median of 6. No clear change (+0.5%).

```diff
diff --git a/include/psnerf_hip.h b/include/psnerf_hip.h
--- a/include/psnerf_hip.h
+++ b/include/psnerf_hip.h
@@ -267,6 +267,42 @@
 int psn_pair_sums_group(int n_items, const PsnPairSumsItem* items, int V, int64_t Ns, int C, const float* pe_l, int64_t ld_pe, int n_pe,
                         int64_t ld_w, float* workspace, void* stream);
 
+#define PSN_SIDE_COLSUM 1
+#define PSN_SIDE_PAIR 2
+#define PSN_WGRAD_MAX_SIDES 4
+#define PSN_SIDE_MAX_UNITS 64
+typedef struct {
+    int kind;
+    const float* X; int64_t ldx;
+    const float* w; int64_t ldw; int n_w;
+    int64_t M; int N;
+    float* out; float* wsum;
+    int accumulate;
+    int n_layers;
+    PsnPairSumsItem layers[PSN_PAIR_GROUP_MAX];
+    int V; int64_t Ns; int C;
+    const float* pe_l; int64_t ld_pe; int n_pe; int64_t ld_w;
+} PsnWgradSide;
+typedef struct {
+    int cus, side_cus;
+    int tile_blocks, side_blocks;
+    int split_big, k_chunk_big;
+    int rblocks, finish_blocks;
+    int64_t workspace_floats;
+    int64_t tile_off[PSN_GEMM_TN_MAX_ITEMS];
+    int64_t tile_cs_off[PSN_GEMM_TN_MAX_ITEMS];
+    int side_start[PSN_WGRAD_MAX_SIDES + 1];
+    int fin_start[PSN_WGRAD_MAX_SIDES + 1];
+    int side_units[PSN_WGRAD_MAX_SIDES];
+    int64_t side_rows[PSN_WGRAD_MAX_SIDES];
+    int64_t side_off[PSN_WGRAD_MAX_SIDES];
+    int64_t side_w_off[PSN_WGRAD_MAX_SIDES];
+} PsnWgradSidesPlan;
+int psn_wgrad_sides_plan(int n_items, const PsnGemmTnItem* items, int64_t K, int n_sides, const PsnWgradSide* sides, int cus,
+                         int side_cus, int split_big, int64_t workspace_addr, PsnWgradSidesPlan* plan);
+int psn_wgrad_sides(int n_items, const PsnGemmTnItem* items, int64_t K, int n_sides, const PsnWgradSide* sides, int side_cus,
+                    int split_big, float* workspace, int64_t workspace_floats, void* stream);
+
 #define PSN_ROW_ADAM_MAX 4
 typedef struct {
     float* param; const float* grad; float* exp_avg; float* exp_avg_sq;
diff --git a/psnerf_amd/csrc/gemm.hip b/psnerf_amd/csrc/gemm.hip
--- a/psnerf_amd/csrc/gemm.hip
+++ b/psnerf_amd/csrc/gemm.hip
@@ -1,4 +1,5 @@
 #include "common.h"
+#include "side_sums.h"
 
 namespace psn {
 
@@ -366,13 +367,7 @@
 }
 
 constexpr int T256 = 256, T256_LD = T256 + 4, TK = 32, T256_BUF = 2 * TK * T256_LD;
-__global__ __launch_bounds__(256, 1) void gemm_tn256_grouped_kernel(GroupedArgs gg) {
-    extern __shared__ __attribute__((aligned(16))) float lds256[];
-    int gi = 0;
-    while (gi + 1 < gg.n && (int64_t)blockIdx.x >= gg.block_start[gi + 1]) ++gi;
-    const GemmArgs g = gg.g[gi];
-    const int split = (int)((int64_t)blockIdx.x - gg.block_start[gi]);
-    if (split >= g.split_k) return;
+__device__ __forceinline__ void tile256_body(const GemmArgs& g, const int split, float* lds256) {
     const int tid = threadIdx.x;
     const int lane = tid & 63, wave = tid >> 6;
     const int wr = wave >> 1, wc = wave & 1;
@@ -555,6 +550,15 @@
                 if (row < g.M && col < g.N) Cw[(int64_t)row * g.N + col] = acc[i][n][r];
             }
         }
+}
+__global__ __launch_bounds__(256, 1) void gemm_tn256_grouped_kernel(GroupedArgs gg) {
+    extern __shared__ __attribute__((aligned(16))) float lds256[];
+    int gi = 0;
+    while (gi + 1 < gg.n && (int64_t)blockIdx.x >= gg.block_start[gi + 1]) ++gi;
+    const GemmArgs g = gg.g[gi];
+    const int split = (int)((int64_t)blockIdx.x - gg.block_start[gi]);
+    if (split >= g.split_k) return;
+    tile256_body(g, split, lds256);
 }
 
 typedef __bf16 gbf16x8 __attribute__((ext_vector_type(8)));
@@ -852,10 +856,7 @@
 struct GroupedReduceArgs {
     ReduceItem it[kMaxGroup];
 };
-__global__ __launch_bounds__(256) void grouped_reduce_kernel(GroupedReduceArgs ra) {
-    const ReduceItem r = ra.it[blockIdx.y];
-    __shared__ float4 red[8][32];
-    const int b = blockIdx.x;
+__device__ __forceinline__ void grouped_reduce_block(const ReduceItem& r, const int b, float4 (*red)[32]) {
     if (b < r.blocks) {
         if (r.vec) {
             const int tx = threadIdx.x & 31, tz = threadIdx.x >> 5;
@@ -904,6 +905,10 @@
             r.colsum[m] = s;
         }
     }
+}
+__global__ __launch_bounds__(256) void grouped_reduce_kernel(GroupedReduceArgs ra) {
+    __shared__ float4 red[8][32];
+    grouped_reduce_block(ra.it[blockIdx.y], blockIdx.x, red);
 }
 
 __global__ __launch_bounds__(256) void splitk_reduce_kernel(const float* __restrict__ ws, int64_t MN, int N,
@@ -982,45 +987,14 @@
                                                                  int64_t ldw, int64_t M, int N, int64_t ldx,
                                                                  int64_t rows_per_block, float* __restrict__ partial) {
     constexpr int NW1 = NW > 0 ? NW : 1;
-    __shared__ float4 red[3][NW1][64];
-    const int c4 = (threadIdx.x & 63) * 4, rsub = threadIdx.x >> 6;
+    __shared__ float4 red[3 * NW1 * 64];
     const int64_t r0 = (int64_t)blockIdx.x * rows_per_block;
     const int64_t r1 = min(M, r0 + rows_per_block);
-    float4 s[NW1];
-#pragma unroll
-    for (int j = 0; j < NW1; ++j) s[j] = make_float4(0.f, 0.f, 0.f, 0.f);
-    if (c4 < N) {
-#pragma unroll 4
-        for (int64_t m = r0 + rsub; m < r1; m += 4) {
-            const float4 x = *reinterpret_cast<const float4*>(X + m * ldx + c4);
-#pragma unroll
-            for (int j = 0; j < NW1; ++j) {
-                const float wj = NW > 0 ? w[m * ldw + j] : 1.0f;
-                if (NW > 0) { s[j].x += wj * x.x; s[j].y += wj * x.y; s[j].z += wj * x.z; s[j].w += wj * x.w; }
-                else { s[j].x += x.x; s[j].y += x.y; s[j].z += x.z; s[j].w += x.w; }
-            }
-        }
-    }
-    if (rsub > 0) {
-#pragma unroll
-        for (int j = 0; j < NW1; ++j) red[rsub - 1][j][threadIdx.x & 63] = s[j];
-    }
-    __syncthreads();
-    if (rsub == 0 && c4 < N) {
-#pragma unroll
-        for (int j = 0; j < NW1; ++j) {
-            const float4 a = red[0][j][threadIdx.x], b = red[1][j][threadIdx.x], c = red[2][j][threadIdx.x];
-            float4 t;
-            t.x = (s[j].x + a.x) + (b.x + c.x); t.y = (s[j].y + a.y) + (b.y + c.y);
-            t.z = (s[j].z + a.z) + (b.z + c.z); t.w = (s[j].w + a.w) + (b.w + c.w);
-            *reinterpret_cast<float4*>(partial + ((int64_t)blockIdx.x * NW1 + j) * N + c4) = t;
-        }
-    }
-}
-__global__ __launch_bounds__(256) void colsum_final_kernel(const float* __restrict__ partial, int nblocks, int N, int NW,
-                                                           int accumulate, float* __restrict__ out) {
-    __shared__ float red[4];
-    const int j = blockIdx.x / N, n = blockIdx.x % N;
+    colsum_vec_block<NW, false>(X, w, ldw, N, ldx, r0, r1, partial + (int64_t)blockIdx.x * NW1 * N, nullptr, red, nullptr);
+}
+__device__ __forceinline__ void colsum_final_block(const float* __restrict__ partial, int nblocks, int N, int NW, int accumulate,
+                                                   float* __restrict__ out, const int blk, float* red) {
+    const int j = blk / N, n = blk % N;
     float s = 0.0f;
     for (int b = threadIdx.x; b < nblocks; b += 256) s += partial[((int64_t)b * NW + j) * N + n];
 #pragma unroll
@@ -1029,7 +1003,144 @@
     __syncthreads();
     if (threadIdx.x == 0) {
         float tot = (red[0] + red[1]) + (red[2] + red[3]);
-        out[blockIdx.x] = accumulate ? out[blockIdx.x] + tot : tot;
+        out[blk] = accumulate ? out[blk] + tot : tot;
+    }
+}
+__global__ __launch_bounds__(256) void colsum_final_kernel(const float* __restrict__ partial, int nblocks, int N, int NW,
+                                                           int accumulate, float* __restrict__ out) {
+    __shared__ float red[4];
+    colsum_final_block(partial, nblocks, N, NW, accumulate, out, blockIdx.x, red);
+}
+
+struct SideDev {
+    int kind, nw, C, V;
+    int64_t ld0, ld1, rows, rpu;
+    float* part;
+    float* wpart;
+    const float* src[PSN_PAIR_GROUP_MAX];
+    float* sx[PSN_PAIR_GROUP_MAX];
+    int units;
+};
+struct WgradSidesArgs {
+    GroupedArgs gg;
+    int T, n_sides;
+    int side_start[PSN_WGRAD_MAX_SIDES + 1];
+    SideDev s[PSN_WGRAD_MAX_SIDES];
+};
+static_assert(sizeof(WgradSidesArgs) <= 4096, "kernel arguments are limited to 4 KB");
+__global__ __launch_bounds__(256, 1) void wgrad_sides_kernel(WgradSidesArgs a) {
+    extern __shared__ __attribute__((aligned(16))) float lds256[];
+    if ((int)blockIdx.x < a.T) {
+        int gi = 0;
+        while (gi + 1 < a.gg.n && (int64_t)blockIdx.x >= a.gg.block_start[gi + 1]) ++gi;
+        const GemmArgs g = a.gg.g[gi];
+        const int split = (int)((int64_t)blockIdx.x - a.gg.block_start[gi]);
+        if (split >= g.split_k) return;
+        tile256_body(g, split, lds256);
+        return;
+    }
+    const int sb = (int)blockIdx.x - a.T;
+    int si = 0;
+    while (si + 1 < a.n_sides && sb >= a.side_start[si + 1]) ++si;
+    if (sb >= a.side_start[a.n_sides]) return;
+    const SideDev& s = a.s[si];
+    const int u = sb - a.side_start[si];
+    float4* red = reinterpret_cast<float4*>(lds256);
+    double* wred = reinterpret_cast<double*>(lds256 + 3 * 4 * 64 * 4);
+    if (s.kind == PSN_SIDE_COLSUM) {
+        const int64_t r0 = (int64_t)u * s.rpu, r1 = min(s.rows, r0 + s.rpu);
+        float* dst = s.part + (int64_t)u * s.nw * s.C;
+        float* wdst = s.wpart + (int64_t)u * s.nw * 2;
+        switch (s.nw) {
+            case 1: colsum_vec_block<1, true>(s.src[0], s.src[1], s.ld1, s.C, s.ld0, r0, r1, dst, wdst, red, wred); break;
+            case 2: colsum_vec_block<2, true>(s.src[0], s.src[1], s.ld1, s.C, s.ld0, r0, r1, dst, wdst, red, wred); break;
+            case 3: colsum_vec_block<3, true>(s.src[0], s.src[1], s.ld1, s.C, s.ld0, r0, r1, dst, wdst, red, wred); break;
+            default: colsum_vec_block<4, true>(s.src[0], s.src[1], s.ld1, s.C, s.ld0, r0, r1, dst, wdst, red, wred); break;
+        }
+    } else {
+        const int layer = u / s.units, ch = u - layer * s.units;
+        const int64_t n0 = (int64_t)ch * s.rpu, n1 = min(s.rows, n0 + s.rpu);
+        float* dst = s.part + (((int64_t)layer * s.units + ch) * s.V) * s.C;
+        pair_sums_block<true>(s.src[layer], s.sx[layer], dst, s.V, s.rows, s.C, n0, n1, reinterpret_cast<float4 (*)[64]>(red));
+    }
+}
+
+struct SideFin {
+    int kind, nw, C, V, units, n_layers, n_pe, accumulate;
+    const float* part; const float* wpart;
+    float* out; float* wsum;
+    const float* pe_l; int64_t ld_pe, ld_w;
+    float* dWl[PSN_PAIR_GROUP_MAX]; float* bias[PSN_PAIR_GROUP_MAX];
+};
+struct WgradFinishArgs {
+    GroupedReduceArgs ra;
+    int n_items, rblocks, n_sides;
+    int fin_start[PSN_WGRAD_MAX_SIDES + 1];
+    SideFin s[PSN_WGRAD_MAX_SIDES];
+};
+static_assert(sizeof(WgradFinishArgs) <= 4096, "kernel arguments are limited to 4 KB");
+__global__ __launch_bounds__(256) void wgrad_finish_kernel(WgradFinishArgs a) {
+    __shared__ float4 red[8][32];
+    __shared__ float dzl[PSN_PAIR_SUMS_MAX_V][64];
+    __shared__ float pel[PSN_PAIR_SUMS_MAX_V][64];
+    const int nred = a.n_items * a.rblocks;
+    if ((int)blockIdx.x < nred) {
+        grouped_reduce_block(a.ra.it[blockIdx.x / a.rblocks], blockIdx.x % a.rblocks, red);
+        return;
+    }
+    const int fb = (int)blockIdx.x - nred;
+    int si = 0;
+    while (si + 1 < a.n_sides && fb >= a.fin_start[si + 1]) ++si;
+    if (a.n_sides == 0 || fb >= a.fin_start[a.n_sides]) return;
+    const SideFin& s = a.s[si];
+    const int b = fb - a.fin_start[si];
+    if (s.kind == PSN_SIDE_COLSUM) {
+        if (b < s.nw * s.C) {
+            colsum_final_block(s.part, s.units, s.C, s.nw, s.accumulate, s.out, b, reinterpret_cast<float*>(red));
+        } else if ((int)threadIdx.x < s.nw) {
+            double t = 0.0;
+            for (int u = 0; u < s.units; ++u) {
+                const float* hl = s.wpart + ((int64_t)u * s.nw + threadIdx.x) * 2;
+                t += (double)hl[0] + (double)hl[1];
+            }
+            s.wsum[threadIdx.x] = (float)t;
+        }
+        return;
+    }
+    const int groups = (s.C + 63) / 64;
+    const int layer = b / groups, c0 = (b - layer * groups) * 64;
+    const int cl = threadIdx.x & 63, slot = threadIdx.x >> 6;
+    const int V = s.V, C = s.C;
+    for (int v = slot; v < PSN_PAIR_SUMS_MAX_V; v += 4) {
+        float t = 0.0f;
+        if (v < V && c0 + cl < C) {
+            const float* p = s.part + ((int64_t)layer * s.units * V + v) * C + c0 + cl;
+            const int64_t step = (int64_t)V * C;
+            int ch = 0;
+            for (; ch + 4 <= s.units; ch += 4) {
+                const float t0 = p[(int64_t)ch * step], t1 = p[(int64_t)(ch + 1) * step], t2 = p[(int64_t)(ch + 2) * step], t3 = p[(int64_t)(ch + 3) * step];
+                t += t0; t += t1; t += t2; t += t3;
+            }
+            for (; ch < s.units; ++ch) t += p[(int64_t)ch * step];
+        }
+        dzl[v][cl] = t;
+        pel[v][cl] = (v < V && cl < s.n_pe) ? s.pe_l[(int64_t)v * s.ld_pe + cl] : 0.0f;
+    }
+    __syncthreads();
+    float* dWl = s.dWl[layer];
+    for (int e = threadIdx.x; e < 64 * s.n_pe; e += 256) {
+        const int c = e / s.n_pe, k = e - c * s.n_pe;
+        if (c0 + c < C) {
+            float w = 0.0f;
+            for (int u = 0; u < V; ++u) w += dzl[u][c] * pel[u][k];
+            dWl[(int64_t)(c0 + c) * s.ld_w + k] = w;
+        }
+    }
+    float* bias = s.bias[layer];
+    if (bias != nullptr && threadIdx.x < 64 && c0 + (int)threadIdx.x < C) {
+        float bsum = 0.0f;
+        for (int u = 0; u < V; ++u) bsum += dzl[u][threadIdx.x];
+        bias[c0 + threadIdx.x] = bsum;
     }
 }
 
@@ -1398,3 +1509,211 @@
     PSN_CHECK_LAUNCH("colsum final");
     return PSN_OK;
 }
+
+static int wgrad_default_side_cus(int cus) { return cus / 8; }
+
+static int wgrad_sides_plan(int n_items, const PsnGemmTnItem* items, int64_t K, int n_sides, const PsnWgradSide* sides, int cus,
+                            int side_cus, int split_req, uintptr_t workspace, PsnWgradSidesPlan* p, PsnGemmTnPlan* tp) {
+    using namespace psn;
+    PSN_CHECK_ARG(n_items >= 0 && n_items <= kMaxGroup && n_sides >= 0 && n_sides <= PSN_WGRAD_MAX_SIDES && n_items + n_sides > 0,
+                  "wgrad_sides: n_items=%d (0..%d), n_sides=%d (0..%d), not both 0", n_items, kMaxGroup, n_sides, PSN_WGRAD_MAX_SIDES);
+    PSN_CHECK_ARG((n_items == 0 || items) && (n_sides == 0 || sides), "wgrad_sides: null item list");
+    PSN_CHECK_ARG(cus > 0, "wgrad_sides: cus=%d", cus);
+    PSN_CHECK_ARG((workspace & 15) == 0, "wgrad_sides: workspace must be 16-byte aligned");
+    *p = PsnWgradSidesPlan{};
+    int products = 0;
+    if (n_items > 0) {
+        const int rc = gemm_tn_plan(n_items, items, K, 1, workspace, tp);
+        if (rc != PSN_OK) return rc;
+        for (int i = 0; i < n_items; ++i) {
+            PSN_CHECK_ARG(tp->kind[i] == PSN_TN_BIG, "wgrad_sides: item %d is not a 256 x 256-tile product (128 < M, N <= 256, aligned, no table)", i);
+            products += items[i].A2 ? 2 : 1;
+        }
+    }
+    for (int i = 0; i < n_sides; ++i) {
+        const PsnWgradSide& s = sides[i];
+        if (s.kind == PSN_SIDE_COLSUM) {
+            PSN_CHECK_ARG(s.X && s.w && s.out && s.wsum, "wgrad_sides: side %d (column sum) has a null pointer", i);
+            PSN_CHECK_ARG(s.n_w >= 1 && s.n_w <= 4 && s.ldw >= s.n_w && s.M >= 1 && s.M < (1ll << 40), "wgrad_sides: side %d n_w=%d M=%lld", i, s.n_w, (long long)s.M);
+            PSN_CHECK_ARG(s.N >= 4 && s.N <= 256 && s.N % 4 == 0 && s.ldx % 4 == 0 && s.ldx >= s.N && ((uintptr_t)s.X & 15) == 0,
+                          "wgrad_sides: side %d needs N <= 256, N %% 4 == 0, ldx %% 4 == 0 and a 16-byte aligned X", i);
+        } else if (s.kind == PSN_SIDE_PAIR) {
+            PSN_CHECK_ARG(s.pe_l && s.n_layers >= 1 && s.n_layers <= PSN_PAIR_GROUP_MAX, "wgrad_sides: side %d (pair sums) n_layers=%d", i, s.n_layers);
+            PSN_CHECK_ARG(s.V >= 1 && s.V <= PSN_PAIR_SUMS_MAX_V && s.C >= 4 && s.C <= 256 && s.C % 4 == 0 && s.Ns >= 1 && s.Ns < (1ll << 40),
+                          "wgrad_sides: side %d V=%d C=%d", i, s.V, s.C);
+            PSN_CHECK_ARG(s.n_pe >= 1 && s.n_pe <= 64 && s.ld_pe >= s.n_pe && s.ld_w >= s.n_pe, "wgrad_sides: side %d n_pe=%d", i, s.n_pe);
+            for (int l = 0; l < s.n_layers; ++l)
+                PSN_CHECK_ARG(s.layers[l].x && s.layers[l].sx && s.layers[l].dWl && (((uintptr_t)s.layers[l].x | (uintptr_t)s.layers[l].sx) & 15) == 0,
+                              "wgrad_sides: side %d layer %d", i, l);
+        } else {
+            PSN_CHECK_ARG(false, "wgrad_sides: side %d has unknown kind %d", i, s.kind);
+        }
+    }
+    int r = (n_sides == 0 || n_items == 0) ? 0 : (side_cus < 0 ? wgrad_default_side_cus(cus) : side_cus);
+    if (r > cus - products) r = cus - products > 0 ? cus - products : 0;
+    p->cus = cus; p->side_cus = r;
+    int split = 1, kc = 0;
+    if (products > 0) {
+        int64_t want = split_req > 0 ? split_req : (cus - r) / products;
+        if (want < 1) want = 1;
+        if (split_req <= 0 && want > K / 256) want = K / 256 > 0 ? K / 256 : 1;
+        if (want > K) want = K;
+        kc = (int)((K + want - 1) / want);
+        kc = ((kc + TK - 1) / TK) * TK;
+        split = (int)((K + kc - 1) / kc);
+    }
+    p->split_big = split; p->k_chunk_big = kc;
+    int64_t off = 0, T = 0;
+    int rblocks = 1;
+    for (int i = 0; i < n_items; ++i) {
+        const PsnGemmTnItem& it = items[i];
+        const int64_t MN = (int64_t)it.M * it.N;
+        const int nseg = it.A2 ? 2 : 1;
+        tp->splits[i] = split * nseg;
+        tp->c_vec[i] = (it.N % 4 == 0) && (MN % 4 == 0);
+        tp->reduce_vec[i] = tp->c_vec[i] && (it.ldc % 4 == 0) && (((uintptr_t)it.C & 15) == 0);
+        p->tile_off[i] = off;
+        off = (off + MN * split * nseg + 3) / 4 * 4;
+        p->tile_cs_off[i] = it.colsum_a ? off : -1;
+        if (it.colsum_a) off = (off + (int64_t)split * it.M + 3) / 4 * 4;
+        T += split * nseg;
+        const int rb = (int)(tp->reduce_vec[i] ? (MN + 127) / 128 : (MN + 255) / 256) + (it.colsum_a ? (it.M + 255) / 256 : 0);
+        if (rb > rblocks) rblocks = rb;
+    }
+    p->tile_blocks = (int)T;
+    p->rblocks = n_items > 0 ? rblocks : 0;
+    int S = 0, F = 0;
+    for (int i = 0; i < n_sides; ++i) {
+        const PsnWgradSide& s = sides[i];
+        p->side_start[i] = S; p->fin_start[i] = F;
+        p->side_off[i] = off;
+        if (s.kind == PSN_SIDE_COLSUM) {
+            int64_t units = (s.M + 127) / 128;
+            if (units > PSN_SIDE_MAX_UNITS) units = PSN_SIDE_MAX_UNITS;
+            p->side_units[i] = (int)units;
+            p->side_rows[i] = (s.M + units - 1) / units;
+            off = (off + units * s.n_w * s.N + 3) / 4 * 4;
+            p->side_w_off[i] = off;
+            off = (off + units * s.n_w * 2 + 3) / 4 * 4;
+            S += (int)units;
+            F += s.n_w * s.N + 1;
+        } else {
+            int64_t rows = ((s.Ns + PSN_SIDE_MAX_UNITS - 1) / PSN_SIDE_MAX_UNITS + 15) / 16 * 16;
+            const int64_t units = (s.Ns + rows - 1) / rows;
+            p->side_units[i] = (int)units;
+            p->side_rows[i] = rows;
+            p->side_w_off[i] = -1;
+            off = (off + (int64_t)s.n_layers * units * s.V * s.C + 3) / 4 * 4;
+            S += (int)units * s.n_layers;
+            F += s.n_layers * ((s.C + 63) / 64);
+        }
+    }
+    p->side_start[n_sides] = S; p->fin_start[n_sides] = F;
+    p->side_blocks = S;
+    p->finish_blocks = n_items * p->rblocks + F;
+    p->workspace_floats = off;
+    return PSN_OK;
+}
+
+extern "C" int psn_wgrad_sides_plan(int n_items, const PsnGemmTnItem* items, int64_t K, int n_sides, const PsnWgradSide* sides, int cus,
+                                    int side_cus, int split_big, int64_t workspace_addr, PsnWgradSidesPlan* plan) {
+    PSN_CHECK_ARG(plan, "wgrad_sides_plan: null plan");
+    PsnGemmTnPlan tp;
+    return wgrad_sides_plan(n_items, items, K, n_sides, sides, cus, side_cus, split_big, (uintptr_t)workspace_addr, plan, &tp);
+}
+
+static int device_cus(int* cus) {
+    static int cached[64] = {0};
+    int dev = 0;
+    if (hipGetDevice(&dev) != hipSuccess || dev < 0 || dev >= 64) { psn::set_error("wgrad_sides: no current device"); return PSN_E_LAUNCH; }
+    if (cached[dev] == 0) {
+        int n = 0;
+        if (hipDeviceGetAttribute(&n, hipDeviceAttributeMultiprocessorCount, dev) != hipSuccess || n <= 0) {
+            psn::set_error("wgrad_sides: cannot read the compute-unit count");
+            return PSN_E_LAUNCH;
+        }
+        cached[dev] = n;
+    }
+    *cus = cached[dev];
+    return PSN_OK;
+}
+
+extern "C" int psn_wgrad_sides(int n_items, const PsnGemmTnItem* items, int64_t K, int n_sides, const PsnWgradSide* sides, int side_cus,
+                               int split_big, float* workspace, int64_t workspace_floats, void* stream) {
+    using namespace psn;
+    PSN_CHECK_ARG(workspace, "wgrad_sides: null workspace");
+    int cus = 0;
+    int rc = device_cus(&cus);
+    if (rc != PSN_OK) return rc;
+    PsnWgradSidesPlan pl;
+    PsnGemmTnPlan tp;
+    rc = wgrad_sides_plan(n_items, items, K, n_sides, sides, cus, side_cus, split_big, (uintptr_t)workspace, &pl, &tp);
+    if (rc != PSN_OK) return rc;
+    PSN_CHECK_ARG(pl.workspace_floats <= workspace_floats, "wgrad_sides: workspace too small (%lld floats needed)", (long long)pl.workspace_floats);
+    WgradSidesArgs a;
+    WgradFinishArgs f;
+    a.gg.n = n_items; a.T = pl.tile_blocks; a.n_sides = n_sides;
+    f.n_items = n_items; f.rblocks = pl.rblocks > 0 ? pl.rblocks : 1; f.n_sides = n_sides;
+    int64_t blocks = 0;
+    for (int i = 0; i < n_items; ++i) {
+        const PsnGemmTnItem& it = items[i];
+        GemmArgs& g = a.gg.g[i];
+        g.M = it.M; g.N = it.N; g.K = (int)(it.k_rows > 0 ? it.k_rows : K); g.A = it.A; g.lda = it.lda; g.B = it.B; g.ldb = it.ldb;
+        g.A2 = it.A2; g.lda2 = it.lda2; g.B2 = it.B2; g.ldb2 = it.ldb2;
+        g.b_div = g.b_mod = 0; g.Bt2 = nullptr; g.ldbt2 = 0; g.b2_div = g.b2_mod = g.b_split = 0;
+        g.bias = nullptr; g.epi = PSN_EPI_NONE; g.aux_in = g.aux_in2 = nullptr; g.aux_out = nullptr;
+        g.ld_aux_in = g.ld_aux_in2 = g.ld_aux_out = 0;
+        g.tiles_n = 1; g.n_tiles = 1;
+        g.k_chunk = pl.k_chunk_big;
+        g.split_k = tp.splits[i];
+        g.seg_splits = pl.split_big;
+        g.a_vec = tp.a_vec[i]; g.b_vec = tp.b_vec[i];
+        g.auxin_vec = g.auxin2_vec = g.auxout_vec = 0;
+        const int64_t MN = (int64_t)it.M * it.N;
+        g.C = workspace + pl.tile_off[i];
+        g.ldc = it.N;
+        g.split_stride = MN;
+        g.c_vec = tp.c_vec[i];
+        g.colsum = it.colsum_a ? workspace + pl.tile_cs_off[i] : nullptr;
+        ReduceItem& r = f.ra.it[i];
+        r.ws = g.C; r.cs_ws = g.colsum; r.C = it.C; r.colsum = it.colsum_a; r.MN = MN; r.ldc = it.ldc; r.N = it.N; r.M = it.M;
+        r.splits = g.split_k; r.cs_splits = pl.split_big; r.accumulate = it.accumulate ? 1 : 0;
+        r.vec = tp.reduce_vec[i];
+        r.blocks = (int)(r.vec ? (MN + 127) / 128 : (MN + 255) / 256);
+        a.gg.block_start[i] = blocks;
+        blocks += g.split_k;
+    }
+    a.gg.block_start[n_items] = blocks;
+    for (int i = 0; i <= n_sides; ++i) { a.side_start[i] = pl.side_start[i]; f.fin_start[i] = pl.fin_start[i]; }
+    for (int i = 0; i < n_sides; ++i) {
+        const PsnWgradSide& s = sides[i];
+        SideDev& d = a.s[i];
+        SideFin& e = f.s[i];
+        d = SideDev{}; e = SideFin{};
+        d.kind = e.kind = s.kind;
+        d.units = e.units = pl.side_units[i];
+        d.rpu = pl.side_rows[i];
+        d.part = workspace + pl.side_off[i];
+        e.part = d.part;
+        if (s.kind == PSN_SIDE_COLSUM) {
+            d.nw = e.nw = s.n_w; d.C = e.C = s.N; d.ld0 = s.ldx; d.ld1 = s.ldw; d.rows = s.M;
+            d.src[0] = s.X; d.src[1] = s.w;
+            d.wpart = workspace + pl.side_w_off[i];
+            e.wpart = d.wpart; e.out = s.out; e.wsum = s.wsum; e.accumulate = s.accumulate ? 1 : 0;
+        } else {
+            d.C = e.C = s.C; d.V = e.V = s.V; d.rows = s.Ns;
+            e.n_layers = s.n_layers; e.n_pe = s.n_pe; e.pe_l = s.pe_l; e.ld_pe = s.ld_pe; e.ld_w = s.ld_w;
+            for (int l = 0; l < s.n_layers; ++l) {
+                d.src[l] = s.layers[l].x; d.sx[l] = s.layers[l].sx;
+                e.dWl[l] = s.layers[l].dWl; e.bias[l] = s.layers[l].bias;
+            }
+        }
+    }
+    PSN_CHECK_ARG(blocks == pl.tile_blocks && blocks + pl.side_blocks < (1ll << 31), "wgrad_sides: too many blocks");
+    hipStream_t st = (hipStream_t)stream;
+    hipLaunchKernelGGL(wgrad_sides_kernel, dim3((unsigned)(pl.tile_blocks + pl.side_blocks)), dim3(256), T256_BUF * 2 * sizeof(float), st, a);
+    PSN_CHECK_LAUNCH("wgrad_sides");
+    hipLaunchKernelGGL(wgrad_finish_kernel, dim3((unsigned)pl.finish_blocks), dim3(256), 0, st, f);
+    PSN_CHECK_LAUNCH("wgrad_sides finish");
+    return PSN_OK;
+}
diff --git a/psnerf_amd/csrc/loss.hip b/psnerf_amd/csrc/loss.hip
--- a/psnerf_amd/csrc/loss.hip
+++ b/psnerf_amd/csrc/loss.hip
@@ -1,4 +1,5 @@
 #include "common.h"
+#include "side_sums.h"
 
 namespace psn {
 
@@ -129,44 +130,10 @@
                        int slices; float* part2; };
 __global__ __launch_bounds__(256) void pair_group_sums_kernel(PairGroupArgs a) {
     const PsnPairSumsItem it = a.it[blockIdx.y];
-    const int V = a.V, C = a.C;
-    const int64_t Ns = a.Ns;
-    const int cg = threadIdx.x & 63, rl = threadIdx.x >> 6;
-    const int64_t n0 = (int64_t)blockIdx.x * a.rows_per_block, n1 = min(Ns, n0 + a.rows_per_block);
-    const bool live = 4 * cg < C;
-    float4 sl[PSN_PAIR_SUMS_MAX_V];
-#pragma unroll
-    for (int v = 0; v < PSN_PAIR_SUMS_MAX_V; ++v) sl[v] = make_float4(0.f, 0.f, 0.f, 0.f);
-    if (live) {
-        for (int64_t n = n0 + rl; n < n1; n += 4) {
-            float4 acc = make_float4(0.f, 0.f, 0.f, 0.f);
-#pragma unroll
-            for (int v = 0; v < PSN_PAIR_SUMS_MAX_V; ++v) {
-                if (v < V) {
-                    const float4 t = *reinterpret_cast<const float4*>(it.x + ((int64_t)v * Ns + n) * C + 4 * cg);
-                    acc.x += t.x; acc.y += t.y; acc.z += t.z; acc.w += t.w;
-                    sl[v].x += t.x; sl[v].y += t.y; sl[v].z += t.z; sl[v].w += t.w;
-                }
-            }
-            *reinterpret_cast<float4*>(it.sx + n * C + 4 * cg) = acc;
-        }
-    }
+    const int64_t n0 = (int64_t)blockIdx.x * a.rows_per_block, n1 = min(a.Ns, n0 + a.rows_per_block);
     __shared__ float4 red[3][64];
-    float* dst = a.part + (((int64_t)blockIdx.y * a.chunks + blockIdx.x) * V) * C;
-#pragma unroll
-    for (int v = 0; v < PSN_PAIR_SUMS_MAX_V; ++v) {
-        if (v < V) {
-            __syncthreads();
-            if (rl > 0) red[rl - 1][cg] = sl[v];
-            __syncthreads();
-            if (rl == 0 && live) {
-                float4 t = sl[v];
-#pragma unroll
-                for (int q = 0; q < 3; ++q) { const float4 o = red[q][cg]; t.x += o.x; t.y += o.y; t.z += o.z; t.w += o.w; }
-                *reinterpret_cast<float4*>(dst + (int64_t)v * C + 4 * cg) = t;
-            }
-        }
-    }
+    float* dst = a.part + (((int64_t)blockIdx.y * a.chunks + blockIdx.x) * a.V) * a.C;
+    pair_sums_block<false>(it.x, it.sx, dst, a.V, a.Ns, a.C, n0, n1, red);
 }
 __global__ __launch_bounds__(1024) void pair_group_final_kernel(PairGroupArgs a) {
     const PsnPairSumsItem it = a.it[blockIdx.y];
diff --git a/psnerf_amd/csrc/side_sums.h b/psnerf_amd/csrc/side_sums.h
--- /dev/null
+++ b/psnerf_amd/csrc/side_sums.h
@@ -0,0 +1,196 @@
+#pragma once
+#include "common.h"
+
+namespace psn {
+
+constexpr int kPairFold = 4;
+constexpr int kColsumFold = 32;
+
+__device__ __forceinline__ void add4(float4& d, const float4& t) { d.x += t.x; d.y += t.y; d.z += t.z; d.w += t.w; }
+
+template <int VT>
+__device__ __forceinline__ void pair_rows_fold(const float* __restrict__ x, float* __restrict__ sx, int64_t Ns, int C, int64_t n0,
+                                               int64_t n1, int cg, int rl, float4 (&sl)[PSN_PAIR_SUMS_MAX_V],
+                                               float4 (&sl2)[PSN_PAIR_SUMS_MAX_V]) {
+    int64_t n = n0 + rl;
+    for (; n + 4 * (kPairFold - 1) < n1; n += 4 * kPairFold) {
+        float4 t[kPairFold][VT];
+#pragma unroll
+        for (int u = 0; u < kPairFold; ++u)
+#pragma unroll
+            for (int v = 0; v < VT; ++v) t[u][v] = *reinterpret_cast<const float4*>(x + ((int64_t)v * Ns + n + 4 * u) * C + 4 * cg);
+#pragma unroll
+        for (int u = 0; u < kPairFold; ++u) {
+            float4 acc = make_float4(0.f, 0.f, 0.f, 0.f);
+#pragma unroll
+            for (int v = 0; v < VT; ++v) { add4(acc, t[u][v]); add4(sl[v], t[u][v]); }
+            *reinterpret_cast<float4*>(sx + (n + 4 * u) * C + 4 * cg) = acc;
+        }
+#pragma unroll
+        for (int v = 0; v < VT; ++v) { add4(sl2[v], sl[v]); sl[v] = make_float4(0.f, 0.f, 0.f, 0.f); }
+    }
+    for (; n < n1; n += 4) {
+        float4 acc = make_float4(0.f, 0.f, 0.f, 0.f);
+#pragma unroll
+        for (int v = 0; v < VT; ++v) {
+            const float4 t = *reinterpret_cast<const float4*>(x + ((int64_t)v * Ns + n) * C + 4 * cg);
+            add4(acc, t); add4(sl[v], t);
+        }
+        *reinterpret_cast<float4*>(sx + n * C + 4 * cg) = acc;
+    }
+}
+
+template <bool FOLD>
+__device__ __forceinline__ void pair_sums_block(const float* __restrict__ x, float* __restrict__ sx, float* __restrict__ dst,
+                                                int V, int64_t Ns, int C, int64_t n0, int64_t n1, float4 (*red)[64]) {
+    const int cg = threadIdx.x & 63, rl = threadIdx.x >> 6;
+    const bool live = 4 * cg < C;
+    float4 sl[PSN_PAIR_SUMS_MAX_V], sl2[FOLD ? PSN_PAIR_SUMS_MAX_V : 1];
+#pragma unroll
+    for (int v = 0; v < PSN_PAIR_SUMS_MAX_V; ++v) sl[v] = make_float4(0.f, 0.f, 0.f, 0.f);
+    if (FOLD) {
+#pragma unroll
+        for (int v = 0; v < PSN_PAIR_SUMS_MAX_V; ++v) sl2[FOLD ? v : 0] = make_float4(0.f, 0.f, 0.f, 0.f);
+    }
+    if (live && FOLD && V == 8) {
+        pair_rows_fold<8>(x, sx, Ns, C, n0, n1, cg, rl, sl, reinterpret_cast<float4 (&)[PSN_PAIR_SUMS_MAX_V]>(sl2));
+    } else if (live) {
+        int it = 0;
+        for (int64_t n = n0 + rl; n < n1; n += 4) {
+            float4 acc = make_float4(0.f, 0.f, 0.f, 0.f);
+#pragma unroll
+            for (int v = 0; v < PSN_PAIR_SUMS_MAX_V; ++v) {
+                if (v < V) {
+                    const float4 t = *reinterpret_cast<const float4*>(x + ((int64_t)v * Ns + n) * C + 4 * cg);
+                    acc.x += t.x; acc.y += t.y; acc.z += t.z; acc.w += t.w;
+                    sl[v].x += t.x; sl[v].y += t.y; sl[v].z += t.z; sl[v].w += t.w;
+                }
+            }
+            *reinterpret_cast<float4*>(sx + n * C + 4 * cg) = acc;
+            if (FOLD && ++it == kPairFold) {
+                it = 0;
+#pragma unroll
+                for (int v = 0; v < PSN_PAIR_SUMS_MAX_V; ++v) {
+                    if (v < V) {
+                        add4(sl2[FOLD ? v : 0], sl[v]);
+                        sl[v] = make_float4(0.f, 0.f, 0.f, 0.f);
+                    }
+                }
+            }
+        }
+    }
+    if (FOLD) {
+#pragma unroll
+        for (int v = 0; v < PSN_PAIR_SUMS_MAX_V; ++v) {
+            add4(sl2[FOLD ? v : 0], sl[v]);
+            sl[v] = sl2[FOLD ? v : 0];
+        }
+    }
+#pragma unroll
+    for (int v = 0; v < PSN_PAIR_SUMS_MAX_V; ++v) {
+        if (v < V) {
+            __syncthreads();
+            if (rl > 0) red[rl - 1][cg] = sl[v];
+            __syncthreads();
+            if (rl == 0 && live) {
+                float4 t = sl[v];
+#pragma unroll
+                for (int q = 0; q < 3; ++q) { const float4 o = red[q][cg]; t.x += o.x; t.y += o.y; t.z += o.z; t.w += o.w; }
+                *reinterpret_cast<float4*>(dst + (int64_t)v * C + 4 * cg) = t;
+            }
+        }
+    }
+}
+
+template <int NW, bool FOLD>
+__device__ __forceinline__ void colsum_vec_block(const float* __restrict__ X, const float* __restrict__ w, int64_t ldw, int N,
+                                                 int64_t ldx, int64_t r0, int64_t r1, float* __restrict__ dst,
+                                                 float* __restrict__ wsum_dst, float4* red_raw, double* wred) {
+    constexpr int NW1 = NW > 0 ? NW : 1;
+    float4 (*red)[NW1][64] = reinterpret_cast<float4 (*)[NW1][64]>(red_raw);
+    const int c4 = (threadIdx.x & 63) * 4, rsub = threadIdx.x >> 6;
+    float4 s[NW1], s2[NW1];
+    double ws[NW1];
+#pragma unroll
+    for (int j = 0; j < NW1; ++j) {
+        s[j] = s2[j] = make_float4(0.f, 0.f, 0.f, 0.f);
+        ws[j] = 0.0;
+    }
+    if (c4 < N) {
+        int64_t m = r0 + rsub;
+        if (FOLD) {
+            for (; m + 4 * (kColsumFold - 1) < r1; m += 4 * kColsumFold) {
+                float4 x[kColsumFold];
+                float wv[kColsumFold][NW1];
+#pragma unroll
+                for (int u = 0; u < kColsumFold; ++u) {
+                    x[u] = *reinterpret_cast<const float4*>(X + (m + 4 * u) * ldx + c4);
+#pragma unroll
+                    for (int j = 0; j < NW1; ++j) wv[u][j] = NW > 0 ? w[(m + 4 * u) * ldw + j] : 1.0f;
+                }
+#pragma unroll
+                for (int u = 0; u < kColsumFold; ++u)
+#pragma unroll
+                    for (int j = 0; j < NW1; ++j) {
+                        const float wj = wv[u][j];
+                        if (NW > 0) { s[j].x += wj * x[u].x; s[j].y += wj * x[u].y; s[j].z += wj * x[u].z; s[j].w += wj * x[u].w; }
+                        else { s[j].x += x[u].x; s[j].y += x[u].y; s[j].z += x[u].z; s[j].w += x[u].w; }
+                        ws[j] += (double)wj;
+                    }
+#pragma unroll
+                for (int j = 0; j < NW1; ++j) {
+                    add4(s2[j], s[j]);
+                    s[j] = make_float4(0.f, 0.f, 0.f, 0.f);
+                }
+            }
+        }
+#pragma unroll 4
+        for (; m < r1; m += 4) {
+            const float4 x = *reinterpret_cast<const float4*>(X + m * ldx + c4);
+#pragma unroll
+            for (int j = 0; j < NW1; ++j) {
+                const float wj = NW > 0 ? w[m * ldw + j] : 1.0f;
+                if (NW > 0) { s[j].x += wj * x.x; s[j].y += wj * x.y; s[j].z += wj * x.z; s[j].w += wj * x.w; }
+                else { s[j].x += x.x; s[j].y += x.y; s[j].z += x.z; s[j].w += x.w; }
+                if (FOLD) ws[j] += (double)wj;
+            }
+        }
+    }
+    if (FOLD) {
+#pragma unroll
+        for (int j = 0; j < NW1; ++j) {
+            add4(s2[j], s[j]);
+            s[j] = s2[j];
+        }
+    }
+    if (rsub > 0) {
+#pragma unroll
+        for (int j = 0; j < NW1; ++j) red[rsub - 1][j][threadIdx.x & 63] = s[j];
+        if (FOLD && (threadIdx.x & 63) == 0) {
+#pragma unroll
+            for (int j = 0; j < NW1; ++j) wred[(rsub - 1) * NW1 + j] = ws[j];
+        }
+    }
+    __syncthreads();
+    if (rsub == 0 && c4 < N) {
+#pragma unroll
+        for (int j = 0; j < NW1; ++j) {
+            const float4 a = red[0][j][threadIdx.x], b = red[1][j][threadIdx.x], c = red[2][j][threadIdx.x];
+            float4 t;
+            t.x = (s[j].x + a.x) + (b.x + c.x); t.y = (s[j].y + a.y) + (b.y + c.y);
+            t.z = (s[j].z + a.z) + (b.z + c.z); t.w = (s[j].w + a.w) + (b.w + c.w);
+            *reinterpret_cast<float4*>(dst + (int64_t)j * N + c4) = t;
+        }
+        if (FOLD && threadIdx.x == 0) {
+#pragma unroll
+            for (int j = 0; j < NW1; ++j) {
+                const double t = (ws[j] + wred[j]) + (wred[NW1 + j] + wred[2 * NW1 + j]);
+                const float hi = (float)t;
+                wsum_dst[2 * j] = hi;
+                wsum_dst[2 * j + 1] = (float)(t - (double)hi);
+            }
+        }
+    }
+}
+
+}
diff --git a/psnerf_amd/hip.py b/psnerf_amd/hip.py
--- a/psnerf_amd/hip.py
+++ b/psnerf_amd/hip.py
@@ -964,6 +964,130 @@
     return out
 
 
+_cu_count = {}
+
+
+def cu_count(device):
+    di = device.index if device.index is not None else torch._C._cuda_getDevice()
+    if di not in _cu_count:
+        _cu_count[di] = int(torch.cuda.get_device_properties(di).multi_processor_count)
+    return _cu_count[di]
+
+
+def wgrad_sides_split(n_products, K, cus, side_cus, split_big=0):
+    if n_products == 0:
+        return 0, 1
+    r = min(side_cus, max(cus - n_products, 0))
+    want = split_big if split_big > 0 else max(1, min((cus - r) // n_products, K // 256 if K >= 256 else 1))
+    want = max(1, min(want, K))
+    kc = (-(-K // want) + 31) // 32 * 32
+    return r, -(-K // kc)
+
+
+def wgrad_sides_workspace(shapes, K, split_big, sides):
+    pad = lambda n: (n + 3) // 4 * 4
+    off = 0
+    for M, N, products, has_cs in shapes:
+        off = pad(off + M * N * split_big * products)
+        if has_cs:
+            off = pad(off + split_big * M)
+    for s in sides:
+        if s[0] == 'colsum':
+            _, M, N, n_w = s
+            units = min(-(-M // 128), SIDE_MAX_UNITS)
+            off = pad(off + units * n_w * N)
+            off = pad(off + units * n_w * 2)
+        else:
+            _, n_layers, V, Ns, C = s
+            rows = (-(-Ns // SIDE_MAX_UNITS) + 15) // 16 * 16
+            off = pad(off + n_layers * (-(-Ns // rows)) * V * C)
+    return off
+
+
+def _wgrad_sides_args(items, colsum_side, pair_side, ptr, outputs):
+    K = items[0]['A'].shape[0] if items else 0
+    arr = (PsnGemmTnItem * max(len(items), 1))()
+    tiles, shapes = [], []
+    for e, it in zip(arr, items):
+        M, N = _tn_shape(it, K)
+        _tn_fill(e, it, K, ptr)
+        dev = it['A'].device
+        C = it.get('out')
+        if C is None and outputs:
+            C = torch.empty(M, N, device=dev, dtype=torch.float32)
+        cs = torch.empty(M, device=dev, dtype=torch.float32) if (it.get('colsum') and outputs) else None
+        e.C, e.ldc = (ptr(C, 'out'), _ld(C)) if C is not None else (16, N)
+        e.colsum_a = (cs.data_ptr() if cs is not None else 16) if it.get('colsum') else None
+        tiles.append((C, cs))
+        shapes.append((M, N, 2 if it.get('A2') is not None else 1, bool(it.get('colsum'))))
+    sides = (PsnWgradSide * WGRAD_MAX_SIDES)()
+    n_sides, mirror, cs_res, pair_res = 0, [], None, None
+    if colsum_side is not None:
+        X, w = colsum_side['X'], colsum_side['w']
+        M, N = X.shape
+        w2 = w if w.dim() == 2 else w.reshape(M, 1)
+        assert w2.shape[0] == M and w2.stride(1) == 1 and 1 <= w2.shape[1] <= 4
+        n_w = w2.shape[1]
+        out = colsum_side.get('out')
+        if out is None and outputs:
+            out = torch.empty(n_w, N, device=X.device, dtype=torch.float32)
+        wsum = torch.empty(n_w, device=X.device, dtype=torch.float32) if outputs else None
+        e = sides[n_sides]
+        n_sides += 1
+        e.kind, e.X, e.ldx, e.w, e.ldw, e.n_w, e.M, e.N = SIDE_COLSUM, ptr(X, 'X'), _ld(X), ptr(w2, 'w'), w2.stride(0), n_w, M, N
+        e.out, e.wsum = (out.data_ptr(), wsum.data_ptr()) if outputs else (16, 16)
+        e.accumulate = int(bool(colsum_side.get('accumulate')))
+        mirror.append(('colsum', M, N, n_w))
+        cs_res = (out, wsum)
+    if pair_side is not None:
+        xs, V, Ns, pe_l = pair_side['xs'], pair_side['V'], pair_side['Ns'], pair_side['pe_l']
+        C = xs[0].shape[1]
+        assert 1 <= len(xs) <= PAIR_GROUP_MAX and all(x.shape == (V * Ns, C) and x.is_contiguous() for x in xs)
+        assert pe_l.stride(1) == 1 and pe_l.shape[0] == V
+        e = sides[n_sides]
+        n_sides += 1
+        e.kind, e.n_layers, e.V, e.Ns, e.C = SIDE_PAIR, len(xs), V, Ns, C
+        e.pe_l, e.ld_pe, e.n_pe, e.ld_w = ptr(pe_l, 'pe_l'), pe_l.stride(0), int(pair_side['n_pe']), 64
+        pair_res = []
+        for l, (x, wb) in enumerate(zip(xs, pair_side['want_bias'])):
+            dev = x.device
+            sx = torch.empty(Ns, C, device=dev, dtype=torch.float32) if outputs else None
+            dWl = torch.empty(C, 64, device=dev, dtype=torch.float32) if outputs else None
+            b = torch.empty(C, device=dev, dtype=torch.float32) if (wb and outputs) else None
+            e.layers[l].x = ptr(x, 'x')
+            e.layers[l].sx, e.layers[l].dWl = (sx.data_ptr(), dWl.data_ptr()) if outputs else (16, 16)
+            e.layers[l].bias = (b.data_ptr() if outputs else 16) if wb else None
+            pair_res.append((sx, dWl, b))
+        mirror.append(('pair', len(xs), V, Ns, C))
+    return K, arr, sides, n_sides, (tiles, cs_res, pair_res), shapes, mirror
+
+
+def wgrad_sides_plan(items, colsum_side=None, pair_side=None, cus=256, side_cus=-1, split_big=0, workspace_addr=0):
+    K, arr, sides, n_sides, _res, _shapes, _mirror = _wgrad_sides_args(items, colsum_side, pair_side, lambda t, name: t.data_ptr(), False)
+    pl = PsnWgradSidesPlan()
+    _check(_lib.psn_wgrad_sides_plan(len(items), ctypes.addressof(arr), K, n_sides, ctypes.addressof(sides), cus, side_cus, split_big,
+                                     workspace_addr, ctypes.addressof(pl)), 'wgrad_sides_plan')
+    return pl
+
+
+WGRAD_SIDE_CUS = -1
+
+
+def wgrad_sides(items, colsum_side=None, pair_side=None, side_cus=None, split_big=0):
+    assert len(items) <= GEMM_TN_MAX_ITEMS
+    K, arr, sides, n_sides, res, shapes, mirror = _wgrad_sides_args(items, colsum_side, pair_side, _mat_ptr, True)
+    dev = (items[0]['A'] if items else (colsum_side['X'] if colsum_side is not None else pair_side['xs'][0])).device
+    side_cus = WGRAD_SIDE_CUS if side_cus is None else side_cus
+    n_products = sum(s[2] for s in shapes)
+    _r, split = wgrad_sides_split(n_products, K, cu_count(dev), 0, split_big)
+    ws = workspace(wgrad_sides_workspace(shapes, K, split, mirror) + 16, dev)
+    flops = sum(2.0 * (arr[i].k_rows or K) * arr[i].M * arr[i].N * shapes[i][2] for i in range(len(items)))
+    with _Prof('gemm_tn_grouped', flops):
+        _check(_lib.psn_wgrad_sides(len(items), ctypes.addressof(arr), K, n_sides, ctypes.addressof(sides), side_cus, split_big,
+                                    ws.data_ptr(), ws.numel(), _stream()), 'wgrad_sides')
+    return res
+
+
 def mlp_pack_layer(W, n_mt, k_tiles, dst, transpose=False):
     assert W.dim() == 2 and W.stride(1) == 1 and W.is_cuda and W.dtype == torch.float32
     rows, cols = (W.shape[1], W.shape[0]) if transpose else (W.shape[0], W.shape[1])
diff --git a/psnerf_amd/ops.py b/psnerf_amd/ops.py
--- a/psnerf_amd/ops.py
+++ b/psnerf_amd/ops.py
@@ -551,6 +551,7 @@
 
 
 RELU_SIGN_BITS = True
+WGRAD_SIDES = True
 
 
 def _sign_bits(rows, n, device):
@@ -616,8 +617,6 @@
         DZ = [torch.empty(Q, 256, device=g.device) for _ in range(n - 1)]
         chain(None, Q, a_div=1, a_mod=Q, rank_init=(g.reshape(Q, 1), Ws[n - 1].reshape(1, -1).contiguous()),
               mask=[(bits if bits is not None else H)[n - 2 - j] for j in range(n - 1)], save=DZ, save_row0=0)
-        grads[2 * (n - 1)] = hip.colsum(H[n - 2], row_weight=g)
-        grads[2 * (n - 1) + 1] = _rowsum_small(g)
         items = []
         where = []
         xl = {}
@@ -635,7 +634,26 @@
                     dWl = hip.gemm(dz_l, pe_lv.contiguous(), trans_a=True)
                     xl[li] = [dz_x, dWl, dz_l.sum(0) if li == 0 else None]
         grouped = [li for li in sorted(xl) if xl[li] is None]
-        if grouped:
+        sides = (WGRAD_SIDES and not hip.WGRAD_X3 and grouped and items and len(items) <= hip.GEMM_TN_MAX_ITEMS
+                 and len(grouped) <= hip.PAIR_GROUP_MAX and all(hip._tn_is_big(it) for it in items))
+        parts = {}
+        if sides:
+            pl = pe_lv.contiguous()
+            tiles, (dw_last, sum_g), pairs = hip.wgrad_sides(
+                items, dict(X=H[n - 2], w=g),
+                dict(xs=[DZ[n - 2 - li] for li in grouped], V=V, Ns=Ns, pe_l=pl, n_pe=pl.shape[1], want_bias=[li == 0 for li in grouped]))
+            grads[2 * (n - 1)], grads[2 * (n - 1) + 1] = dw_last, sum_g
+            for li, r in zip(grouped, pairs):
+                xl[li] = list(r)
+            for (li, kind), (C, cs) in zip(where, tiles):
+                parts[(li, kind)] = C
+                if cs is not None:
+                    grads[2 * li + 1] = cs
+            items = []
+        else:
+            grads[2 * (n - 1)] = hip.colsum(H[n - 2], row_weight=g)
+            grads[2 * (n - 1) + 1] = _rowsum_small(g)
+        if grouped and not sides:
             pl = pe_lv.contiguous()
             for li, r in zip(grouped, hip.pair_sums_group([DZ[n - 2 - li] for li in grouped], V, Ns, pl, pl.shape[1],
                                                           [li == 0 for li in grouped])):
@@ -643,7 +661,6 @@
         lis = sorted(xl)
         for li, (C, _cs) in zip(lis, hip.gemm_tn_grouped([dict(A=xl[li][0], B=pe_x) for li in lis])):
             xl[li][0] = C
-        parts = {}
         if items:
             for (li, kind), (C, cs) in zip(where, hip.gemm_tn_grouped(items)):
                 parts[(li, kind)] = C
diff --git a/psnerf_amd/stage2/renderer.py b/psnerf_amd/stage2/renderer.py
--- a/psnerf_amd/stage2/renderer.py
+++ b/psnerf_amd/stage2/renderer.py
@@ -276,6 +276,9 @@
         def ones3(b=1):
             return _Dense(1.0, b, 3)
 
+        inv_early = None
+        if ns > 0 and idx.is_cuda and idx.dtype == torch.int64:
+            inv_early = hip.inverse_index(idx.contiguous(), n_pix, count=input.get('surface_count'))
         surf = gather(points).contiguous()
         out_n = {}
         normal_s = None
@@ -466,7 +469,9 @@
         with_rows = [v for v in lazy.values() if v.rows is not None]
         done = {}
         if with_rows:
-            if idx.is_cuda and idx.dtype == torch.int64:
+            if inv_early is not None:
+                inv = inv_early
+            elif idx.is_cuda and idx.dtype == torch.int64:
                 inv = hip.inverse_index(idx.contiguous(), n_pix, count=input.get('surface_count'))
             else:
                 inv = torch.full((n_pix,), -1, dtype=torch.int32, device=device)
```
